# langtech-bsc/quantool

Measured on AMD Instinct MI355X. Metric: quantized weights/sec (GPTQ int4, Llama-3-8B, 512 calib samples), higher is better.
Workload: dtype f32

## Files before the change

include/quantool_amd.h:

```cpp
#ifndef QUANTOOL_AMD_H
#define QUANTOOL_AMD_H

#include <stddef.h>
#include <stdint.h>

#ifdef __cplusplus
extern "C" {
#endif

typedef void* qt_stream_t;

enum qt_status {
    QT_OK = 0,
    QT_ERR_INVALID = -1,
    QT_ERR_NOT_PD = -2,
    QT_ERR_WORKSPACE = -3,
    QT_ERR_HIP = -4,
    QT_ERR_UNSUPPORTED = -5
};

enum qt_dtype { QT_F32 = 0, QT_BF16 = 1, QT_F16 = 2 };

int qt_version(void);
const char* qt_last_error(void);

size_t qt_xtx_workspace_bytes(int64_t n_tokens, int K);
int qt_xtx_accumulate(const void* X, int x_dtype, int64_t n_tokens, int K, int64_t ldx, float* G,
                      void* workspace, size_t workspace_bytes, qt_stream_t stream);

size_t qt_xtx_accumulate_f32_workspace_bytes(int64_t n_tokens, int K);
int qt_xtx_accumulate_f32(const float* X, int64_t n_tokens, int K, int64_t ldx, float* G, void* workspace,
                          size_t workspace_bytes, qt_stream_t stream);

size_t qt_act_stats_workspace_bytes(int64_t n_tokens, int K);
int qt_act_stats_accumulate(const void* X, int x_dtype, int64_t n_tokens, int K, int64_t ldx, float* abs_sum,
                            float* cmin, float* cmax, void* workspace, size_t workspace_bytes,
                            qt_stream_t stream);

size_t qt_hessian_prepare_workspace_bytes(int K);
int qt_hessian_prepare(const float* G, int K, int64_t n_samples, float percdamp,
                       const int32_t* perm, float* A, uint8_t* dead, float* diag_out,
                       void* workspace, size_t workspace_bytes, qt_stream_t stream);
int qt_hessian_prepare_damp(const float* G, int K, int64_t n_samples, float percdamp,
                            const int32_t* perm, float* A, uint8_t* dead, float* diag_out, float* damp_out,
                            void* workspace, size_t workspace_bytes, qt_stream_t stream);
int qt_hessian_diag(const float* G, int K, int64_t n_samples, float* diag_out, qt_stream_t stream);
int qt_argsort_desc(const float* values, int K, int32_t* perm, int32_t* inv, qt_stream_t stream);

size_t qt_cholesky_inverse_upper_workspace_bytes(int K);
int qt_cholesky_inverse_upper(float* A, int K, float* U, int32_t* info, void* workspace,
                              size_t workspace_bytes, qt_stream_t stream);

size_t qt_cholesky_inverse_upper_batched_workspace_bytes(int K, int n_problems);
int qt_cholesky_inverse_upper_batched(float* A, int64_t strideA, int K, float* U, int64_t strideU, int32_t* info,
                                      int n_problems, void* workspace, size_t workspace_bytes, qt_stream_t stream);

int qt_cholesky_inverse_upper_bounded(float* A, int K, float* U, int32_t* info, const float* min_eig_lb,
                                      void* workspace, size_t workspace_bytes, qt_stream_t stream);
int qt_cholesky_inverse_upper_batched_bounded(float* A, int64_t strideA, int K, float* U, int64_t strideU, int32_t* info,
                                              int n_problems, const float* min_eig_lb, void* workspace,
                                              size_t workspace_bytes, qt_stream_t stream);

int qt_group_minmax_qparams(const void* W, int w_dtype, int R, int K, int64_t ldw, int group_size,
                            int symmetric, int num_bits, float* scale, float* zp, float* scale_t,
                            float* zp_t, qt_stream_t stream);

int qt_weight_gather_f32(const void* W, int w_dtype, int R, int K, int64_t ldw, const int32_t* perm,
                         const uint8_t* dead, float* W_f32, qt_stream_t stream);

int qt_weight_gather_qparams(const void* W, int w_dtype, int R, int K, int64_t ldw, const int32_t* perm,
                             const uint8_t* dead, int group_size, int symmetric, int num_bits, float* W_f32, float* scale,
                             float* zp, float* scale_t, float* zp_t, int64_t ld_t, qt_stream_t stream);

size_t qt_gptq_sweep_workspace_bytes(int R, int K, int blocksize);
int qt_gptq_sweep(float* W, int R, int K, const float* U, const float* scale_t, const float* zp_t,
                  int G, const int32_t* g_idx, int blocksize, int num_bits, int8_t* Qt,
                  float* loss, void* workspace, size_t workspace_bytes, qt_stream_t stream);

int qt_gptq_sweep_grouped(float* W, int R, int K, const float* U, int64_t strideU, int n_groups, const int32_t* row_end,
                          const float* scale_t, const float* zp_t, int G, const int32_t* g_idx, int blocksize,
                          int num_bits, int8_t* Qt, float* loss, void* workspace, size_t workspace_bytes,
                          qt_stream_t stream);

int qt_pack_int4(const int8_t* Qt, int R, int K, const int32_t* col_src, int32_t* packed,
                 qt_stream_t stream);

int qt_dequantize(const int8_t* Qt, int R, int K, const int32_t* col_src, const float* scale,
                  const float* zp, int G, const int32_t* g_of_col, void* out, int out_dtype,
                  int64_t ldo, qt_stream_t stream);

size_t qt_awq_weight_mean_workspace_bytes(int R, int K);
int qt_awq_weight_mean_accumulate(const void* W, int w_dtype, int R, int K, int64_t ldw, int group_size,
                                  float* w_sum, void* workspace, size_t workspace_bytes,
                                  qt_stream_t stream);
int qt_awq_scales(const float* x_abs_sum, int64_t n_tokens, const float* w_sum, int64_t n_rows, int K,
                  int n_grid, int duo_scaling, float* scales, qt_stream_t stream);
int qt_symmetrize_lower(float* G, int K, qt_stream_t stream);
size_t qt_awq_loss_workspace_bytes(int R, int K);
int qt_awq_loss(const void* W, int w_dtype, int R, int K, int64_t ldw, const float* s, int group_size,
                int symmetric, int num_bits, const float* Gfull, int64_t n_tokens, int exact, float weight,
                int accumulate, float* loss_out, void* workspace, size_t workspace_bytes, qt_stream_t stream);
size_t qt_awq_losses_workspace_bytes(int R, int K, int n_grid);
int qt_awq_losses(const void* W, int w_dtype, int R, int K, int64_t ldw, const float* scales, int n_grid,
                  int group_size, int symmetric, int num_bits, const float* Gfull, int64_t n_tokens, float weight,
                  int accumulate, float* losses, void* workspace, size_t workspace_bytes, qt_stream_t stream);
int qt_argmin_f32(const float* values, int n, int32_t* index_out, qt_stream_t stream);
int qt_awq_pseudo_quantize(const void* W, int w_dtype, int R, int K, int64_t ldw, const float* s, int group_size,
                           int symmetric, int num_bits, void* out, int64_t ldo, qt_stream_t stream);
int qt_scale_columns(const void* W, int w_dtype, int R, int K, int64_t ldw, const float* s, int divide,
                     void* out, int64_t ldo, qt_stream_t stream);
int qt_rtn_quantize(const void* W, int w_dtype, int R, int K, int64_t ldw, const float* scale,
                    const float* zp, int G, int group_size, int num_bits, int8_t* Qt, qt_stream_t stream);

size_t qt_col_absmax_workspace_bytes(int R, int K);
int qt_col_absmax_accumulate(const void* W, int w_dtype, int R, int K, int64_t ldw, float* wmax,
                             void* workspace, size_t workspace_bytes, qt_stream_t stream);
int qt_smoothquant_scales(const float* cmin, const float* cmax, const float* wmax, int K, float alpha,
                          float* s, qt_stream_t stream);

size_t qt_sgemm_tn_f32_workspace_bytes(int M, int N);
int qt_sgemm_tn_f32(const float* A, int64_t lda, const float* B, int64_t ldb, const float* Cin,
                    int64_t ldcin, float* Cout, int64_t ldcout, int M, int N, int kdim, int skip_zero_k,
                    int mode, int allow_split_k, void* workspace, size_t workspace_bytes, qt_stream_t stream);

int qt_xtx_tile_table_check(int K, int* n_tiles_out, int* chunk_panels_out, int* round_panels_out);

size_t qt_xtx_dot_workspace_bytes(int64_t n_tokens, int K);
int qt_xtx_dot(const void* X, int x_dtype, int64_t n_tokens, int K, int64_t ldx, const float* H, double scale,
               float* out, int accumulate, void* workspace, size_t workspace_bytes, qt_stream_t stream);

size_t qt_gemm3_tn_f32_workspace_bytes(int M, int N, int k);
int qt_gemm3_tn_f32(const float* A, int64_t lda, const float* B, int64_t ldb, float* C, int64_t ldc, int M,
                    int N, int k, int kind, void* workspace, size_t workspace_bytes, qt_stream_t stream);
int qt_gemm3_tn_f32_ex(const float* A, int64_t lda, const float* B, int64_t ldb, float* C, int64_t ldc, int M, int N,
                       int k, int kind, int tri, int tight, int batch, int64_t bsA, int64_t bsB, int64_t bsC,
                       void* workspace, size_t workspace_bytes, qt_stream_t stream);

int qt_gemm3_tn_f16x2(const float* A, int64_t lda, const float* B, int64_t ldb, float* C, int64_t ldc, int M, int N,
                      int k, int kind, int tri, int tight, int batch, int64_t bsA, int64_t bsB, int64_t bsC,
                      const float* bound_a, const float* bound_b, void* workspace, size_t workspace_bytes,
                      qt_stream_t stream);

int qt_gemm3_plan_check(int Tm, int Tn, int c_end, int tri, int* n_items_out, int* n_slabs_out, int* longest_out);
enum qt_act { QT_ACT_SILU = 0 };
#define QT_I8_MID_MAX_M 128
#define QT_I8_MID_K_UNIT 128
#define QT_I8_RING_K_UNIT 128
#define QT_I8_RING_SLOTS 8
#define QT_I8_RING_LEAD 6
#define QT_I8_RING_W4_K_UNIT 128
#define QT_I8_RING_W4_SLOTS 8
#define QT_I8_RING_W4_LEAD 6
#define QT_MOE_I8_WIDE_K_UNIT 128
#define QT_MOE_I8_WIDE_TILE_ROWS 128
#define QT_MOE_I8_WIDE_MAX_E 4096
enum qt_weight_format { QT_W_INT8 = 0, QT_W_INT4_PACKED = 1 };
int qt_quantize_tokens_i8(const void* X, int x_dtype, int64_t M, int K, int64_t ldx, const int32_t* col_perm,
                          int symmetric, int8_t* Xq, float* s_x, int32_t* zp_x, qt_stream_t stream);
int qt_act_mul_quantize_i8(const void* gate, int64_t ldg, const void* up, int64_t ldu, int x_dtype, int64_t M, int K,
                           int act, const int32_t* col_perm, int symmetric, int8_t* Xq, float* s_x, int32_t* zp_x,
                           void* H, int64_t ldh, qt_stream_t stream);
int qt_rmsnorm_quantize_i8(const void* X, int64_t ldx, const void* weight, int x_dtype, int64_t M, int K, float eps,
                           const int32_t* col_perm, int symmetric, int8_t* Xq, float* s_x, int32_t* zp_x,
                           void* Y, int64_t ldy, float* rstd, qt_stream_t stream);
int qt_gemm_i8(const int8_t* Xq, int64_t M, int K, const void* Wq, int w_format, int N, const float* s_x,
               const int32_t* zp_x, const float* s_w, int G, const int32_t* wsum, const void* bias, void* Y,
               int out_dtype, int64_t ldy, qt_stream_t stream);
int qt_gemm_i8_skinny(const int8_t* Xq, int M, int K, const void* Wq, int w_format, int N, const float* s_x,
                      const int32_t* zp_x, const float* s_w, int G, const int32_t* wsum, const void* bias, void* Y,
                      int out_dtype, int64_t ldy, qt_stream_t stream);
int qt_gemm_i8_ring(const int8_t* Xq, int64_t M, int K, const void* Wq, int w_format, int N, const float* s_x,
                    const int32_t* zp_x, const float* s_w, int G, const int32_t* wsum, const void* bias, void* Y,
                    int out_dtype, int64_t ldy, qt_stream_t stream);
int qt_gemm_i8_ring_w4(const int8_t* Xq, int64_t M, int K, const void* Wq, int w_format, int N, const float* s_x,
                       const int32_t* zp_x, const float* s_w, int G, const int32_t* wsum, const void* bias, void* Y,
                       int out_dtype, int64_t ldy, qt_stream_t stream);
int qt_gemm_i8_mid(const int8_t* Xq, int64_t M, int K, const void* Wq, int w_format, int N, const float* s_x,
                   const int32_t* zp_x, const float* s_w, int G, const int32_t* wsum, const void* bias, void* Y,
                   int out_dtype, int64_t ldy, qt_stream_t stream);

int qt_moe_route(const void* top_k_index, int index_is_int64, int64_t T, int k, int E, int32_t* offsets,
                 int32_t* src_token, int32_t* src_slot, int32_t* row_of, qt_stream_t stream);
int qt_gemm_i8_grouped(const int8_t* Xq, int K, const int32_t* row_idx, int64_t R, const int32_t* offsets, int E,
                       const void* Wq, int w_format, int N, const float* s_x, const int32_t* zp_x, const float* s_w,
                       int G, const int32_t* wsum, void* Y, int out_dtype, int64_t ldy, qt_stream_t stream);
int qt_gemm_i8_skinny_grouped(const int8_t* Xq, int K, const int32_t* row_idx, int64_t R, const int32_t* offsets,
                              int E, const void* Wq, int w_format, int N, const float* s_x, const int32_t* zp_x,
                              const float* s_w, int G, const int32_t* wsum, void* Y, int out_dtype, int64_t ldy,
                              qt_stream_t stream);
int qt_gemm_i8_ring_grouped(const int8_t* Xq, int K, const int32_t* row_idx, int64_t R, const int32_t* offsets, int E,
                            const void* Wq, int w_format, int N, const float* s_x, const int32_t* zp_x,
                            const float* s_w, int G, const int32_t* wsum, void* Y, int out_dtype, int64_t ldy,
                            int64_t x_rows, qt_stream_t stream);
int qt_moe_gemm_i8_ring_w4(const int8_t* Xq, int K, const int32_t* row_idx, int64_t R, const int32_t* offsets, int E,
                           const void* Wq, int w_format, int N, const float* s_x, const int32_t* zp_x,
                           const float* s_w, int G, const int32_t* wsum, void* Y, int out_dtype, int64_t ldy,
                           int64_t x_rows, qt_stream_t stream);
int qt_moe_gemm_i8_wide(const int8_t* Xq, int K, const int32_t* row_idx, int64_t R, const int32_t* offsets, int E,
                        const void* Wq, int w_format, int N, const float* s_x, const int32_t* zp_x, const float* s_w,
                        int G, const int32_t* wsum, void* Y, int out_dtype, int64_t ldy, int64_t x_rows,
                        qt_stream_t stream);
int qt_moe_combine(const void* Y, int dtype, int H, int64_t ldy, const int32_t* row_of, const float* weights,
                   int64_t T, int k, void* out, qt_stream_t stream);

int qt_dequantize_weight(const void* Wq, int w_format, int N, int K, const float* s_w, int G, const int8_t* zp_w,
                         const int32_t* g_idx, void* W, int dtype, int64_t ldw, qt_stream_t stream);
int qt_gemm_wq_skinny(const void* X, int x_dtype, int M, int K, int64_t ldx, const void* Wq, int w_format, int N,
                      const float* s_w, int G, const int8_t* zp_w, const int32_t* g_idx, const void* bias, void* Y,
                      int64_t ldy, qt_stream_t stream);

int qt_gemm_wq_stream(const void* X, int x_dtype, int M, int K, int64_t ldx, const void* Wq, int w_format, int N,
                      const float* s_w, int G, const int8_t* zp_w, const int32_t* g_idx, const void* bias, void* Y,
                      int64_t ldy, qt_stream_t stream);
#define QT_WQ_STREAM_MAX_M 128
#define QT_WQ_STREAM_K_UNIT 128
#define QT_WQ_STREAM_MAX_LDX 33554432

int qt_gemm_wq_grouped(const void* X, int x_dtype, int K, int64_t ldx, const int32_t* row_idx, int64_t R,
                       const int32_t* offsets, int E, const void* Wq, int w_format, int N, const float* s_w, int G,
                       const int8_t* zp_w, const int32_t* g_idx, void* Y, int64_t ldy, qt_stream_t stream);

int qt_moe_gemm_wq_wide(const void* X, int x_dtype, int K, int64_t ldx, const int32_t* row_idx, int64_t R,
                        const int32_t* offsets, int E, const void* Wq, int w_format, int N, const float* s_w, int G,
                        const int8_t* zp_w, const int32_t* g_idx, void* Y, int64_t ldy, int64_t x_rows,
                        qt_stream_t stream);
#define QT_MOE_WQ_WIDE_K_UNIT 128
#define QT_MOE_WQ_WIDE_MAX_E 4096
#define QT_MOE_WQ_WIDE_MAX_SLOTS 65535

enum qt_prof_kernel { QT_PROF_XTX = 0, QT_PROF_SWEEP_BLOCK = 1, QT_PROF_NUM_KERNELS = 2 };
int qt_profile_enable(int on);
int qt_profile_read(int kernel_id, double* total_ms, int64_t* launches);

#ifdef __cplusplus
}
#endif
#endif
```

quantool_amd/csrc/cholesky.hip:

```cpp
#include <stdlib.h>
#include <string.h>

#include <map>
#include <tuple>
#include <vector>

#include "common.h"
#include "gemm3_tn.h"
#include "sgemm_tn.h"

namespace {

constexpr int NB = 128;
constexpr int NBO_MAX = 1024;
static int chol_block_env(const char* name) {
    const char* e = getenv(name);
    if (!e) return 0;
    int x = atoi(e) / 128 * 128;
    return x < 128 ? 128 : (x > NBO_MAX ? NBO_MAX : x);
}
struct G3Step {
    int n_items = 0, n_red = 0;
    size_t item_off = 0, red_off = 0;
};
struct CholG3Plan {
    bool any = false;
    std::vector<G3Step> fac, inv;
    char* blob = nullptr;
    size_t blob_bytes = 0;
    int max_slabs = 0;
};

static int chol_g3_min_chunks() {
    const char* on = getenv("QT_CHOL_G3");
    if (on && atoi(on) == 0) return 0;
    const char* e = getenv("QT_CHOL_G3_MIN_CHUNKS");
    const int x = e ? atoi(e) : 64;
    return x < 1 ? 1 : x;
}

static int chol_g3_target_items(int K) {
    const char* e = getenv("QT_G3_TARGET_ITEMS");
    if (e && atoi(e) > 0) return atoi(e);
    return K < 8192 ? 96 : 256;
}

static const CholG3Plan* chol_g3_plan(int K, int NBO, int NBI) {
    static std::mutex m;
    static std::map<std::tuple<int, int, int, int>, CholG3Plan*> plans;
    const int min_chunks = chol_g3_min_chunks();
    const int target_items = chol_g3_target_items(K);
    std::lock_guard<std::mutex> lock(m);
    const auto key = std::make_tuple(K, NBO, NBI, min_chunks * 1024 + target_items);
    auto it = plans.find(key);
    if (it != plans.end()) return it->second;
    CholG3Plan* pl = new CholG3Plan();
    std::vector<char> bytes;
    auto add = [&](int Tm, int Tn, int c_end, int tri) {
        G3Step st;
        if (min_chunks <= 0 || K % 8 != 0 || g3_row_chunks(Tm, Tn, c_end, tri) * G3_CHUNK_ROWS < (long)min_chunks * 128) return st;
        std::vector<G3Item> items;
        std::vector<G3Red> red;
        g3_plan_row(Tm, Tn, c_end, tri, items, red, target_items);
        st.n_items = (int)items.size();
        st.n_red = (int)red.size();
        st.item_off = qt_align_up(bytes.size(), 256);
        bytes.resize(st.item_off + items.size() * sizeof(G3Item));
        memcpy(bytes.data() + st.item_off, items.data(), items.size() * sizeof(G3Item));
        st.red_off = qt_align_up(bytes.size(), 256);
        bytes.resize(st.red_off + red.size() * sizeof(G3Red));
        if (!red.empty()) memcpy(bytes.data() + st.red_off, red.data(), red.size() * sizeof(G3Red));
        for (const G3Red& r : red) pl->max_slabs = pl->max_slabs > r.first + r.count ? pl->max_slabs : r.first + r.count;
        pl->any = true;
        return st;
    };
    for (int J0 = 0; J0 < K; J0 += NBO) {
        const int J1 = (K - J0 < NBO) ? K : J0 + NBO;
        pl->fac.push_back(J0 == 0 ? G3Step() : add((J1 - J0 + 255) / 256, (K - J0 + 255) / 256, J0 / G3_CHUNK_ROWS, 0));
    }
    for (int I0 = 0; I0 < K; I0 += NBI) {
        const int I1 = (K - I0 < NBI) ? K : I0 + NBI;
        pl->inv.push_back(I0 == 0 ? G3Step() : add((I1 - I0 + 255) / 256, (I0 + 255) / 256, I0 / G3_CHUNK_ROWS, 1));
    }
    if (pl->any) {
        pl->blob_bytes = qt_align_up(bytes.size(), 256);
        if (hipHostMalloc((void**)&pl->blob, pl->blob_bytes, hipHostMallocDefault) != hipSuccess) {
            pl->any = false;
            pl->blob = nullptr;
        } else {
            memcpy(pl->blob, bytes.data(), bytes.size());
        }
    }
    if (!pl->any) {
        pl->blob_bytes = 0;
        pl->max_slabs = 0;
        for (G3Step& st : pl->fac) st = G3Step();
        for (G3Step& st : pl->inv) st = G3Step();
    }
    plans[key] = pl;
    return pl;
}
static size_t chol_g3_ws_bytes(const CholG3Plan* pl, int K) {
    if (!pl->any) return 0;
    return 2 * qt_align_up((size_t)3 * K * K * 2, 256) + (size_t)pl->max_slabs * 256 * 256 * 4 + pl->blob_bytes + 256;
}

static const CholG3Plan* chol_blocks(int K, int& NBO, int& NBI) {
    const int eo = chol_block_env("QT_CHOL_NBO"), ei = chol_block_env("QT_CHOL_NBI");
    NBO = eo ? eo : 512;
    NBI = ei ? ei : 512;
    const CholG3Plan* pl = chol_g3_plan(K, NBO, NBI);
    if (pl->any) return pl;
    NBO = eo ? eo : 256;
    NBI = ei ? ei : 256;
    return chol_g3_plan(K, NBO, NBI);
}

constexpr int LDP = NB + 1;

constexpr int LDT = NB + 4;
constexpr int RD_STRIDE = NB * NB + 4 * 32 * 32;

#define QT_SEL4(kb, v0, v1, v2, v3) ((kb) == 0 ? (v0) : (kb) == 1 ? (v1) : (kb) == 2 ? (v2) : (v3))

constexpr int LDA = NB + 4;

__device__ __forceinline__ float readlane_f(float v, int lane) {
    return __int_as_float(__builtin_amdgcn_readlane(__float_as_int(v), lane));
}

__device__ __forceinline__ void mma32_tn(const float* A, int lda, const float* B, int ldb, f32x16& acc,
                                         int l31, int h, bool negate_a) {
#pragma unroll
    for (int kk = 0; kk < 16; ++kk) {
        float a = A[(2 * kk + h) * lda + l31];
        const float b = B[(2 * kk + h) * ldb + l31];
        if (negate_a) a = -a;
        acc = __builtin_amdgcn_mfma_f32_32x32x2f32(a, b, acc, 0, 0, 0);
    }
}

constexpr int POTF2_THREADS = 512, POTF2_WAVES = POTF2_THREADS / 64;
__global__ __launch_bounds__(POTF2_THREADS) void potf2_kernel(const float* P, int64_t ldp, int n,
                                                    float* Rout, int64_t ldr,
                                                    float* __restrict__ Rd, int32_t* info, int col0, int prio,
                                                    int64_t bsP, int64_t bsRd) {
    qt_set_chain_prio(prio);
    if (blockIdx.x) {
        P += (size_t)blockIdx.x * bsP;
        Rout += (size_t)blockIdx.x * bsP;
        Rd += (size_t)blockIdx.x * bsRd;
        info += blockIdx.x;
    }
    extern __shared__ __attribute__((aligned(16))) float sm[];
    float* As = sm;
    float* Xs = sm + NB * LDA;
    const int tid = threadIdx.x, lane = tid & 63;
    const int wave = __builtin_amdgcn_readfirstlane(tid >> 6);
    const int l31 = lane & 31, h = lane >> 5;

    if ((ldp & 3) == 0 && (n & 3) == 0 && (((uintptr_t)P) & 15) == 0) {
        constexpr int NV = NB * NB / 4 / POTF2_THREADS;
        f32x4 v[NV];
#pragma unroll
        for (int r = 0; r < NV; ++r) {
            const int e4 = tid + POTF2_THREADS * r;
            const int i = e4 >> 5, j = (e4 & 31) * 4;
            const int ic = i < n ? i : n - 1, jc = j < n ? j : n - 4;
            v[r] = *(const f32x4*)(P + (size_t)ic * ldp + jc);
        }
#pragma unroll
        for (int r = 0; r < NV; ++r) {
            const int e4 = tid + POTF2_THREADS * r;
            const int i = e4 >> 5, j = (e4 & 31) * 4;
            f32x4 x;
#pragma unroll
            for (int q = 0; q < 4; ++q) x[q] = (i < n && j + q < n) ? v[r][q] : (i == j + q ? 1.0f : 0.0f);
            *(f32x4*)(As + i * LDA + j) = x;
        }
    } else {
        for (int e = tid; e < NB * NB; e += POTF2_THREADS) {
            const int i = e / NB, j = e % NB;
            const int lo = i < j ? i : j, hi = i < j ? j : i;
            float v = (i == j) ? 1.0f : 0.0f;
            if (hi < n) v = P[(size_t)lo * ldp + hi];
            As[i * LDA + j] = v;
        }
    }
    __syncthreads();

    int bad = 0;
#pragma unroll 1
    for (int kb = 0; kb < 4; ++kb) {
        float* Akk = As + (32 * kb) * LDA + 32 * kb;
        if (wave == 0) {
            f32x16 c1, c2;
#pragma unroll
            for (int r = 0; r < 16; ++r) {
                const int i = (r & 3) + 8 * (r >> 2) + 4 * h;
                c1[r] = Akk[i * LDA + l31];
                c2[r] = (i == l31) ? 1.0f : 0.0f;
            }
#pragma unroll
            for (int c = 0; c < 32; ++c) {
                const int rc = (c & 3) + 4 * (c >> 3);
                const int hc = (c >> 2) & 1;
                float piv = readlane_f(c1[rc], c + 32 * hc);
                const bool isbad = !(piv > 0.0f);
                bad = (isbad && bad == 0 && 32 * kb + c < n) ? 32 * kb + c + 1 : bad;
                piv = isbad ? 1.0f : piv;
                float rs = __builtin_amdgcn_rsqf(piv);
                rs = rs * fmaf(-0.5f * piv * rs, rs, 1.5f);
                const bool mine = h == hc;
                const float rr = c1[rc] * rs, zz = c2[rc] * rs;
                c1[rc] = mine ? rr : c1[rc];
                c2[rc] = mine ? zz : c2[rc];
                if (c < 31) {
                    const float a = (mine && l31 > c) ? -rr : 0.0f;
                    const float b1 = (mine && l31 >= c) ? rr : 0.0f, b2 = mine ? zz : 0.0f;
                    c1 = __builtin_amdgcn_mfma_f32_32x32x2f32(a, b1, c1, 0, 0, 0);
                    c2 = __builtin_amdgcn_mfma_f32_32x32x2f32(a, b2, c2, 0, 0, 0);
                }
            }
#pragma unroll
            for (int r = 0; r < 16; ++r) {
                const int i = (r & 3) + 8 * (r >> 2) + 4 * h;
                Akk[i * LDA + l31] = (i <= l31) ? c1[r] : 0.0f;
                Xs[(kb * 32 + l31) * 32 + i] = (i >= l31) ? c2[r] : 0.0f;
            }
        }
        __syncthreads();
        if (kb == 3) break;
        for (int a = kb + 1 + wave; a < 4; a += POTF2_WAVES) {
            f32x16 acc;
#pragma unroll
            for (int r = 0; r < 16; ++r) acc[r] = 0.0f;
            float* Bt = As + (32 * kb) * LDA + 32 * a;
            mma32_tn(Xs + kb * 1024, 32, Bt, LDA, acc, l31, h, false);
#pragma unroll
            for (int r = 0; r < 16; ++r) Bt[((r & 3) + 8 * (r >> 2) + 4 * h) * LDA + l31] = acc[r];
        }
        __syncthreads();
        {
            int t = 0;
            for (int a = kb + 1; a < 4; ++a)
                for (int a2 = a; a2 < 4; ++a2, ++t) {
                    if ((t % POTF2_WAVES) != wave) continue;
                    float* Ct = As + (32 * a) * LDA + 32 * a2;
                    f32x16 acc;
#pragma unroll
                    for (int r = 0; r < 16; ++r) acc[r] = Ct[((r & 3) + 8 * (r >> 2) + 4 * h) * LDA + l31];
                    mma32_tn(As + (32 * kb) * LDA + 32 * a, LDA, As + (32 * kb) * LDA + 32 * a2, LDA, acc, l31, h,
                             true);
#pragma unroll
                    for (int r = 0; r < 16; ++r) Ct[((r & 3) + 8 * (r >> 2) + 4 * h) * LDA + l31] = acc[r];
                }
        }
        __syncthreads();
    }
    if (bad != 0 && tid == 0) atomicCAS(info, 0, col0 + bad);
    const bool vec_out = (ldr & 3) == 0 && (n & 3) == 0 && (((uintptr_t)Rout) & 15) == 0;
    for (int e4 = tid; e4 < NB * NB / 4; e4 += POTF2_THREADS) {
        const int i = e4 >> 5, j = (e4 & 31) * 4;
        f32x4 v = *(const f32x4*)(As + i * LDA + j);
#pragma unroll
        for (int q = 0; q < 4; ++q) v[q] = (j + q >= i) ? v[q] : 0.0f;
        *(f32x4*)(Rd + i * NB + j) = v;
        if (i < n && j + 3 >= i && j < n) {
            if (vec_out) {
                *(f32x4*)(Rout + (size_t)i * ldr + j) = v;
            } else {
#pragma unroll
                for (int q = 0; q < 4; ++q)
                    if (j + q >= i && j + q < n) Rout[(size_t)i * ldr + j + q] = v[q];
            }
        }
    }
    for (int e4 = tid; e4 < 4 * 32 * 32 / 4; e4 += POTF2_THREADS) *(f32x4*)(Rd + NB * NB + 4 * e4) = *(const f32x4*)(Xs + 4 * e4);
}

__global__ __launch_bounds__(256) void trsm_rt_kernel(const float* __restrict__ Rd, int n,
                                                      const float* B, int64_t ldb,
                                                      float* Z, int64_t ldz, int ncols, int prio, int64_t bsRd,
                                                      int64_t bsB) {
    qt_set_chain_prio(prio);
    if (blockIdx.y) {
        Rd += (size_t)blockIdx.y * bsRd;
        B += (size_t)blockIdx.y * bsB;
        Z += (size_t)blockIdx.y * bsB;
    }
    extern __shared__ __attribute__((aligned(16))) float Rs[];
    const int tid = threadIdx.x, lane = tid & 63, wave = tid >> 6;
    const float* D32 = Rs + NB * NB;
    const int l31 = lane & 31, h = lane >> 5;
    const int col = blockIdx.x * 128 + wave * 32 + l31;
    const bool cok = col < ncols;
    const int colc = cok ? col : ncols - 1;

    f32x16 acc[4];
#pragma unroll
    for (int a = 0; a < 4; ++a)
#pragma unroll
        for (int r = 0; r < 16; ++r) {
            const int row = 32 * a + (r & 3) + 8 * (r >> 2) + 4 * h;
            acc[a][r] = (row < n) ? B[(size_t)row * ldb + colc] : 0.0f;
        }
    {
        constexpr int NV = RD_STRIDE / 4 / 256;
        static_assert(NV * 4 * 256 == RD_STRIDE, "whole float4s per thread");
        f32x4 v[NV];
#pragma unroll
        for (int r = 0; r < NV; ++r) v[r] = ((const f32x4*)Rd)[tid + 256 * r];
#pragma unroll
        for (int r = 0; r < NV; ++r) ((f32x4*)Rs)[tid + 256 * r] = v[r];
    }
    __syncthreads();

#pragma unroll
    for (int b = 0; b < 4; ++b) {
        f32x16 zb;
#pragma unroll
        for (int r = 0; r < 16; ++r) zb[r] = 0.0f;
#pragma unroll
        for (int r = 0; r < 16; ++r) {
            const int k = (r & 3) + 8 * (r >> 2) + 4 * h;
            const float av = D32[(b * 32 + k) * 32 + l31];
            zb = __builtin_amdgcn_mfma_f32_32x32x2f32(av, acc[b][r], zb, 0, 0, 0);
        }
        acc[b] = zb;
#pragma unroll
        for (int a = b + 1; a < 4; ++a) {
#pragma unroll
            for (int r = 0; r < 16; ++r) {
                const int k = (r & 3) + 8 * (r >> 2) + 4 * h;
                const float av = -Rs[(32 * b + k) * NB + 32 * a + l31];
                acc[a] = __builtin_amdgcn_mfma_f32_32x32x2f32(av, zb[r], acc[a], 0, 0, 0);
            }
        }
    }
    if (cok) {
#pragma unroll
        for (int a = 0; a < 4; ++a)
#pragma unroll
            for (int r = 0; r < 16; ++r) {
                const int row = 32 * a + (r & 3) + 8 * (r >> 2) + 4 * h;
                if (row < n) Z[(size_t)row * ldz + col] = acc[a][r];
            }
    }
}

__global__ __launch_bounds__(128) void trinv_batched_kernel(const float* __restrict__ Rd_all, int K,
                                                            float* __restrict__ Dinv_all,
                                                            float* __restrict__ Y, int64_t ldy, int64_t bsW, int64_t bsY) {
    if (blockIdx.y) {
        Rd_all += (size_t)blockIdx.y * bsW;
        Dinv_all += (size_t)blockIdx.y * bsW;
        Y += (size_t)blockIdx.y * bsY;
    }
    extern __shared__ __attribute__((aligned(16))) float sm[];
    float* Rt = sm;
    float* Xs = sm + NB * LDT;
    const int b = blockIdx.x;
    const int n = (K - b * NB < NB) ? K - b * NB : NB;
    const float* Rd = Rd_all + (size_t)b * RD_STRIDE;
    const int j = threadIdx.x;
    for (int e = j; e < NB * NB; e += NB) {
        const int i = e / NB, c = e % NB;
        Rt[c * LDT + i] = Rd[e];
    }
    __syncthreads();
    float x0[32], x1[32], x2[32], x3[32];
#pragma unroll
    for (int r = 0; r < 32; ++r) {
        x0[r] = (r == j) ? 1.0f : 0.0f;
        x1[r] = (32 + r == j) ? 1.0f : 0.0f;
        x2[r] = (64 + r == j) ? 1.0f : 0.0f;
        x3[r] = (96 + r == j) ? 1.0f : 0.0f;
    }
#pragma unroll 1
    for (int pb = 3; pb >= 0; --pb) {
#pragma unroll
        for (int pp = 31; pp >= 0; --pp) {
            const int p = 32 * pb + pp;
            const float* rp = Rt + p * LDT;
            const float xp = QT_SEL4(pb, x0[pp], x1[pp], x2[pp], x3[pp]) / rp[p];
            if (pb == 0) x0[pp] = xp;
            if (pb == 1) x1[pp] = xp;
            if (pb == 2) x2[pp] = xp;
            if (pb == 3) x3[pp] = xp;
#define QT_XUPD(arr, a, r_to)                                                 \
    _Pragma("unroll") for (int r4 = 0; r4 < (r_to); r4 += 4) {                 \
        const f32x4 v4 = *(const f32x4*)(rp + 32 * (a) + r4);                 \
        _Pragma("unroll") for (int e = 0; e < 4; ++e)                         \
            if (r4 + e < (r_to)) arr[r4 + e] = fmaf(-v4[e], xp, arr[r4 + e]); \
    }
            if (pb == 0) { QT_XUPD(x0, 0, pp) } else { QT_XUPD(x0, 0, 32) }
            if (pb == 1) { QT_XUPD(x1, 1, pp) } else if (pb > 1) { QT_XUPD(x1, 1, 32) }
            if (pb == 2) { QT_XUPD(x2, 2, pp) } else if (pb > 2) { QT_XUPD(x2, 2, 32) }
            if (pb == 3) { QT_XUPD(x3, 3, pp) }
#undef QT_XUPD
        }
    }
#pragma unroll
    for (int r = 0; r < 32; ++r) {
        Xs[r * LDP + j] = x0[r];
        Xs[(32 + r) * LDP + j] = x1[r];
        Xs[(64 + r) * LDP + j] = x2[r];
        Xs[(96 + r) * LDP + j] = x3[r];
    }
    __syncthreads();
    float* Dinv = Dinv_all + (size_t)b * NB * NB;
    float* Yd = Y + (size_t)(b * NB) * ldy + b * NB;
    for (int e = j; e < NB * NB; e += NB) {
        const int i = e / NB, jj = e % NB;
        const bool in = (i < n && jj < n);
        Dinv[e] = (in && jj >= i) ? Xs[i * LDP + jj] : 0.0f;
        if (in) Yd[(size_t)i * ldy + jj] = (jj <= i) ? Xs[jj * LDP + i] : 0.0f;
    }
}

__global__ __launch_bounds__(256) void trinv_mfma_kernel(const float* __restrict__ Rd_all, int K,
                                                         float* __restrict__ Dinv_all,
                                                         float* __restrict__ Y, int64_t ldy, int64_t bsW, int64_t bsY) {
    if (blockIdx.y) {
        Rd_all += (size_t)blockIdx.y * bsW;
        Dinv_all += (size_t)blockIdx.y * bsW;
        Y += (size_t)blockIdx.y * bsY;
    }
    extern __shared__ __attribute__((aligned(16))) float Rs[];
    const int blk = blockIdx.x;
    const int n = (K - blk * NB < NB) ? K - blk * NB : NB;
    const float* Rd = Rd_all + (size_t)blk * RD_STRIDE;
    const int tid = threadIdx.x, lane = tid & 63, wave = tid >> 6;
    {
        constexpr int NV = RD_STRIDE / 4 / 256;
        f32x4 v[NV];
#pragma unroll
        for (int r = 0; r < NV; ++r) v[r] = ((const f32x4*)Rd)[tid + 256 * r];
#pragma unroll
        for (int r = 0; r < NV; ++r) ((f32x4*)Rs)[tid + 256 * r] = v[r];
    }
    const float* D32 = Rs + NB * NB;
    const int l31 = lane & 31, h = lane >> 5;
    const int col = wave * 32 + l31;

    f32x16 acc[4];
#pragma unroll
    for (int a = 0; a < 4; ++a)
#pragma unroll
        for (int r = 0; r < 16; ++r) {
            const int row = 32 * a + (r & 3) + 8 * (r >> 2) + 4 * h;
            acc[a][r] = (row == col) ? 1.0f : 0.0f;
        }
    __syncthreads();

#pragma unroll
    for (int b = 0; b < 4; ++b) {
        f32x16 zb;
#pragma unroll
        for (int r = 0; r < 16; ++r) zb[r] = 0.0f;
#pragma unroll
        for (int r = 0; r < 16; ++r) {
            const int k = (r & 3) + 8 * (r >> 2) + 4 * h;
            const float av = D32[(b * 32 + k) * 32 + l31];
            zb = __builtin_amdgcn_mfma_f32_32x32x2f32(av, acc[b][r], zb, 0, 0, 0);
        }
        acc[b] = zb;
#pragma unroll
        for (int a = b + 1; a < 4; ++a) {
#pragma unroll
            for (int r = 0; r < 16; ++r) {
                const int k = (r & 3) + 8 * (r >> 2) + 4 * h;
                const float av = -Rs[(32 * b + k) * NB + 32 * a + l31];
                acc[a] = __builtin_amdgcn_mfma_f32_32x32x2f32(av, zb[r], acc[a], 0, 0, 0);
            }
        }
    }
    float* Dinv = Dinv_all + (size_t)blk * NB * NB;
    float* Yd = Y + (size_t)(blk * NB) * ldy + blk * NB;
#pragma unroll
    for (int a = 0; a < 4; ++a)
#pragma unroll
        for (int r = 0; r < 16; ++r) {
            const int row = 32 * a + (r & 3) + 8 * (r >> 2) + 4 * h;
            const bool in = row < n && col < n;
            const float z = (in && row >= col) ? acc[a][r] : 0.0f;
            Dinv[col * NB + row] = z;
            if (in) Yd[(size_t)row * ldy + col] = z;
        }
}

__global__ __launch_bounds__(256) void transpose_lower_block_kernel(const float* __restrict__ Y, int64_t ldy, int w,
                                                                    float* __restrict__ XT, int ldx, int64_t bsY,
                                                                    int64_t bsXT) {
    if (blockIdx.z) {
        Y += (size_t)blockIdx.z * bsY;
        XT += (size_t)blockIdx.z * bsXT;
    }
    __shared__ float tile[32][33];
    const int bx = blockIdx.x * 32, by = blockIdx.y * 32;
    const int tx = threadIdx.x & 31, ty = threadIdx.x >> 5;
    for (int r = ty; r < 32; r += 8) {
        const int m = bx + r, k = by + tx;
        tile[r][tx] = (m < w && k < w && k <= m) ? Y[(size_t)m * ldy + k] : 0.0f;
    }
    __syncthreads();
    for (int r = ty; r < 32; r += 8) {
        const int k = by + r, m = bx + tx;
        if (k < w && m < w) XT[(size_t)k * ldx + m] = tile[tx][r];
    }
}

__global__ __launch_bounds__(256) void flat_reverse_lower_to_upper_kernel(float* __restrict__ U, int K, int64_t bsU) {
    U += (size_t)blockIdx.z * bsU;
    const int j = blockIdx.x * blockDim.x + threadIdx.x;
    const int i = blockIdx.y;
    if (j >= K || j < i) return;
    const size_t e = (size_t)i * K + j;
    const size_t pe = (size_t)(K - 1 - i) * K + (K - 1 - j);
    if (i == j) {
        if (e <= pe) {
            const float t = U[e];
            U[e] = U[pe];
            U[pe] = t;
        }
    } else {
        U[e] = U[pe];
        U[pe] = 0.0f;
    }
}

__global__ __launch_bounds__(256) void identity_if_failed_kernel(float* __restrict__ U, int K,
                                                                 const int32_t* __restrict__ info, int64_t bsU) {
    if (info[blockIdx.z] == 0) return;
    U += (size_t)blockIdx.z * bsU;
    for (int i = blockIdx.x; i < K; i += gridDim.x)
        for (int j = threadIdx.x; j < K; j += blockDim.x) U[(size_t)i * K + j] = (i == j) ? 1.0f : 0.0f;
}

__global__ __launch_bounds__(256) void chol_scales_kernel(const float* __restrict__ A, int64_t bsA, int K,
                                                          const float* __restrict__ min_eig_lb, int32_t* __restrict__ e,
                                                          int32_t* __restrict__ info) {
    __shared__ float red[256];
    const int b = blockIdx.x, nprob = gridDim.x;
    const float* Ab = A + (size_t)b * bsA;
    float m = 0.0f;
    for (int i = threadIdx.x; i < K; i += 256) m = fmaxf(m, Ab[(size_t)i * K + i]);
    red[threadIdx.x] = m;
    __syncthreads();
    for (int s = 128; s > 0; s >>= 1) {
        if ((int)threadIdx.x < s) red[threadIdx.x] = fmaxf(red[threadIdx.x], red[threadIdx.x + s]);
        __syncthreads();
    }
    if (threadIdx.x == 0) {
        auto clampe = [](float t) { return (int)fminf(fmaxf(t, (float)-G3_E_MAX), (float)G3_E_MAX); };
        const float d = red[0], lb = min_eig_lb[b];
        e[b] = (d > 0.0f && d < 3.0e38f) ? clampe(3.0f - ceilf(0.5f * log2f(d))) : 0;
        if (lb > 0.0f && lb < 3.0e38f) {
            e[nprob + b] = clampe(3.0f - ceilf(-0.5f * log2f(lb)));
        } else {
            e[nprob + b] = 0;
            info[b] = K + 1;
        }
    }
}

}

static size_t chol_problem_ws_bytes(int K, const CholG3Plan* g3) {
    const size_t nb = (K + NB - 1) / NB;
    const size_t split = (size_t)2048 * NB * NB * 4 + (size_t)NBO_MAX * K * 4;
    size_t n = (size_t)NB * K * 4 + (size_t)NBO_MAX * K * 4 + (size_t)NBO_MAX * NBO_MAX * 4 + nb * (NB * NB + RD_STRIDE) * 4 + split + 256;
    if (g3->any) n += 2 * qt_align_up((size_t)3 * K * K * 2, 256) + (size_t)g3->max_slabs * 256 * 256 * 4 + 256;
    return qt_align_up(n, 256);
}

extern "C" size_t qt_cholesky_inverse_upper_batched_workspace_bytes(int K, int n_problems) {
    if (K <= 0 || n_problems <= 0) return 0;
    int nbo_, nbi_;
    const CholG3Plan* g3 = chol_blocks(K, nbo_, nbi_);
    return (size_t)n_problems * chol_problem_ws_bytes(K, g3) + g3->blob_bytes + 512;
}

extern "C" size_t qt_cholesky_inverse_upper_workspace_bytes(int K) {
    return qt_cholesky_inverse_upper_batched_workspace_bytes(K, 1);
}

static int chol_run(float* A, int64_t strideA, int K, float* U, int64_t strideU, int32_t* info, int nprob, void* workspace,
                    size_t workspace_bytes, hipStream_t stream, const float* min_eig_lb = nullptr) {
    bool f16x2 = min_eig_lb != nullptr;
    if (const char* e = getenv("QT_CHOL_PLANES")) {
        if (strcmp(e, "bf16x3") == 0) f16x2 = false;
        else if (strcmp(e, "f16x2") == 0) {
            QT_CHECK_ARG(min_eig_lb, "qt_cholesky_inverse_upper: QT_CHOL_PLANES=f16x2 needs a bound on lambda_min (the _bounded entry points)");
        } else {
            QT_CHECK_ARG(false, "qt_cholesky_inverse_upper: QT_CHOL_PLANES=%s (bf16x3 | f16x2)", e);
        }
    }
    const size_t need = qt_cholesky_inverse_upper_batched_workspace_bytes(K, nprob);
    if (!workspace || workspace_bytes < need) {
        qt_set_error("qt_cholesky_inverse_upper: workspace %zu < required %zu", workspace_bytes, need);
        return QT_ERR_WORKSPACE;
    }
    const int nblk = (K + NB - 1) / NB;
    char* ws = (char*)qt_align_up((size_t)workspace, 256);
    int NBO, NBI;
    const CholG3Plan* g3 = chol_blocks(K, NBO, NBI);
    const size_t prob_bytes = chol_problem_ws_bytes(K, g3);
    const int64_t sW = (int64_t)(prob_bytes / 4);
    const int64_t sA = nprob > 1 ? strideA : 0, sU = nprob > 1 ? strideU : 0;
    float* T = (float*)ws;
    float* TI = T + (size_t)NB * K;
    float* XT = TI + (size_t)NBO_MAX * K;
    float* Rd = XT + (size_t)NBO_MAX * NBO_MAX;
    float* Dinv = Rd + (size_t)nblk * RD_STRIDE;
    float* split_ws = Dinv + (size_t)nblk * NB * NB;
    const size_t split_ws_bytes = (size_t)2048 * NB * NB * 4 + (size_t)NBO_MAX * K * 4;
    unsigned short *Rpl = nullptr, *Ypl = nullptr;
    float* g3_slabs = nullptr;
    char* g3_tab = nullptr;
    const int64_t plane_stride = (int64_t)K * K;
    if (g3->any) {
        char* q = (char*)qt_align_up((size_t)((char*)split_ws + split_ws_bytes), 256);
        Rpl = (unsigned short*)q;
        q += qt_align_up((size_t)3 * K * K * 2, 256);
        Ypl = (unsigned short*)q;
        q += qt_align_up((size_t)3 * K * K * 2, 256);
        g3_slabs = (float*)q;
        g3_tab = (char*)qt_align_up((size_t)(ws + (size_t)nprob * prob_bytes), 256);
        QT_HIP(hipMemcpyAsync(g3_tab, g3->blob, g3->blob_bytes, hipMemcpyHostToDevice, stream));
    }
    f16x2 = f16x2 && g3->any;
    int32_t* eR = f16x2 ? (int32_t*)(Rpl + 2 * plane_stride) : nullptr;
    int32_t* eY = f16x2 ? eR + nprob : nullptr;
    static_assert(2 * SG_MAX_BATCH * sizeof(int32_t) <= (size_t)NB * NB * 2, "the exponents fit the smallest third plane");
    auto g3_row = [&](const G3Step& st, const unsigned short* Bplanes, int col_a0, int col_b0, int M, int N, float* C,
                      int64_t bsC, int mode) -> int {
        G3Args a;
        a.Apl = Rpl;
        a.Bpl = Bplanes;
        a.plane_stride = plane_stride;
        a.ld = K;
        a.rowA0 = a.rowB0 = 0;
        a.colA0 = col_a0;
        a.colB0 = col_b0;
        a.colmax = K;
        a.M = M;
        a.N = N;
        a.C = C;
        a.ldc = K;
        a.mode = mode;
        a.slabs = g3_slabs;
        a.items = (const G3Item*)(g3_tab + st.item_off);
        a.n_items = st.n_items;
        a.red = (const G3Red*)(g3_tab + st.red_off);
        a.n_red = st.n_red;
        a.batch = nprob;
        a.bsApl = a.bsBpl = sW * 2;
        a.bsC = bsC;
        a.bsSlabs = sW;
        if (f16x2) {
            a.planes = G3_F16X2;
            a.eA = eR;
            a.eB = Bplanes == Rpl ? eR : eY;
        }
        return qt_gemm3_launch(a, stream);
    };
    auto sgemm = [&](SgemmArgs& g, int64_t bsA_, int64_t bsB_, int64_t bsC_) -> int {
        g.batch = nprob;
        g.bsA = bsA_;
        g.bsB = bsB_;
        g.bsCin = g.bsCout = bsC_;
        g.bs_split = sW;
        return qt_sgemm_tn(g, stream);
    };
    float* Y = U;
    const int64_t sY = sU;
    const size_t inv_lds = (size_t)(NB * LDT + NB * LDP) * sizeof(float);
    const size_t potf2_lds = (size_t)(NB * LDA + 4 * 32 * 32) * sizeof(float);
    static QtOncePerDevice lds_attr;
    QT_HIP(lds_attr.run([&] {
        hipError_t e = hipFuncSetAttribute((const void*)potf2_kernel, hipFuncAttributeMaxDynamicSharedMemorySize,
                                           (int)potf2_lds);
        if (e == hipSuccess)
            e = hipFuncSetAttribute((const void*)trsm_rt_kernel, hipFuncAttributeMaxDynamicSharedMemorySize,
                                    (int)(RD_STRIDE * sizeof(float)));
        if (e == hipSuccess)
            e = hipFuncSetAttribute((const void*)trinv_batched_kernel, hipFuncAttributeMaxDynamicSharedMemorySize,
                                    (int)inv_lds);
        if (e == hipSuccess)
            e = hipFuncSetAttribute((const void*)trinv_mfma_kernel, hipFuncAttributeMaxDynamicSharedMemorySize,
                                    (int)(RD_STRIDE * sizeof(float)));
        return e;
    }));
    QT_HIP(hipMemsetAsync(info, 0, sizeof(int32_t) * nprob, stream));
    const int prio = qt_chain_prio();
    if (f16x2) {
        hipLaunchKernelGGL(chol_scales_kernel, dim3(nprob), dim3(256), 0, stream, (const float*)A, sA, K, min_eig_lb, eR, info);
        QT_LAUNCH_CHECK();
    }

    for (int J0 = 0, Jb = 0; J0 < K; J0 += NBO, ++Jb) {
        const int J1 = (K - J0 < NBO) ? K : J0 + NBO;
        if (g3->any && J0 > 0) {
            const G3Step& st = g3->fac[Jb];
            float* C = A + (size_t)J0 * K + J0;
            if (st.n_items > 0) {
                int rc = g3_row(st, Rpl, J0, J0, J1 - J0, K - J0, C, sA, G3_SUB);
                if (rc) return rc;
            } else {
                SgemmArgs g;
                g.A = A + J0; g.lda = K;
                g.B = A + J0; g.ldb = K;
                g.Cin = C; g.ldcin = K;
                g.Cout = C; g.ldcout = K;
                g.M = J1 - J0; g.N = K - J0; g.kdim = J0; g.k_mode = SG_K_FULL; g.mode = SG_MODE_SUB;
                g.split_ws = split_ws; g.split_ws_bytes = split_ws_bytes;
                int rc = sgemm(g, sA, sA, sA);
                if (rc) return rc;
            }
        }
        for (int j0 = J0; j0 < J1; j0 += NB) {
            const int j = j0 / NB, nbj = (K - j0 < NB) ? K - j0 : NB;
            float* Ajj = A + (size_t)j0 * K + j0;
            if (j0 > J0) {
                SgemmArgs g;
                g.A = A + (size_t)J0 * K + j0; g.lda = K;
                g.B = A + (size_t)J0 * K + j0; g.ldb = K;
                g.Cin = Ajj; g.ldcin = K;
                g.Cout = Ajj; g.ldcout = K;
                g.M = nbj; g.N = K - j0; g.kdim = j0 - J0; g.k_mode = SG_K_FULL; g.mode = SG_MODE_SUB;
                int rc = sgemm(g, sA, sA, sA);
                if (rc) return rc;
            }
            hipLaunchKernelGGL(potf2_kernel, dim3(nprob), dim3(POTF2_THREADS), potf2_lds, stream, (const float*)Ajj, (int64_t)K, nbj,
                               Ajj, (int64_t)K, Rd + (size_t)j * RD_STRIDE, info, j0, prio, sA, sW);
            QT_LAUNCH_CHECK();
            const int rest = K - j0 - nbj;
            if (rest > 0) {
                hipLaunchKernelGGL(trsm_rt_kernel, dim3((rest + 127) / 128, nprob), dim3(256), RD_STRIDE * sizeof(float),
                                   stream, (const float*)(Rd + (size_t)j * RD_STRIDE), nbj, (const float*)(Ajj + nbj),
                                   (int64_t)K, Ajj + nbj, (int64_t)K, rest, prio, sW, sA);
                QT_LAUNCH_CHECK();
            }
        }
        const int rem = K - J1;
        if (g3->any) {
            if (rem > 0) {
                int rc = f16x2 ? qt_split2h_launch(A + (size_t)J0 * K + J0, K, J1 - J0, K - J0, Rpl + (size_t)J0 * K + J0, K,
                                                   plane_stride, 0, 0, 0, eR, stream, nprob, sA, sW * 2)
                               : qt_split3_launch(A + (size_t)J0 * K + J0, K, J1 - J0, K - J0, Rpl + (size_t)J0 * K + J0, K,
                                                  plane_stride, 0, 0, 0, stream, nprob, sA, sW * 2);
                if (rc) return rc;
            }
        } else if (rem > 0) {
            SgemmArgs g;
            g.A = A + (size_t)J0 * K + J1; g.lda = K;
            g.B = A + (size_t)J0 * K + J1; g.ldb = K;
            g.Cin = A + (size_t)J1 * K + J1; g.ldcin = K;
            g.Cout = A + (size_t)J1 * K + J1; g.ldcout = K;
            g.M = rem; g.N = rem; g.kdim = J1 - J0; g.k_mode = SG_K_FULL; g.mode = SG_MODE_SUB;
            g.upper_only = 1;
            int rc = sgemm(g, sA, sA, sA);
            if (rc) return rc;
        }
    }
    {
        const char* e = getenv("QT_CHOL_TRINV");
        if (e && strcmp(e, "div") == 0)
            hipLaunchKernelGGL(trinv_batched_kernel, dim3(nblk, nprob), dim3(NB), inv_lds, stream, (const float*)Rd, K, Dinv, Y,
                               (int64_t)K, sW, sY);
        else
            hipLaunchKernelGGL(trinv_mfma_kernel, dim3(nblk, nprob), dim3(256), RD_STRIDE * sizeof(float), stream,
                               (const float*)Rd, K, Dinv, Y, (int64_t)K, sW, sY);
    }
    QT_LAUNCH_CHECK();
    for (int I0 = 0, Ib = 0; I0 < K; I0 += NBI, ++Ib) {
        const int I1 = (K - I0 < NBI) ? K : I0 + NBI;
        const int Wi = I1 - I0;
        for (int i0 = I0 + NB; i0 < I1; i0 += NB) {
            const int i = i0 / NB, nbi = (K - i0 < NB) ? K - i0 : NB;
            SgemmArgs g;
            g.A = A + (size_t)I0 * K + i0; g.lda = K;
            g.B = Y + (size_t)I0 * K + I0; g.ldb = K;
            g.Cin = nullptr; g.ldcin = 0;
            g.Cout = T; g.ldcout = K;
            g.M = nbi; g.N = i0 - I0; g.kdim = i0 - I0; g.k_mode = SG_K_FROM_N0; g.mode = SG_MODE_SET;
            int rc = sgemm(g, sA, sY, sW);
            if (rc) return rc;
            SgemmArgs t;
            t.A = Dinv + (size_t)i * NB * NB; t.lda = NB;
            t.B = T; t.ldb = K;
            t.Cin = nullptr; t.ldcin = 0;
            t.Cout = Y + (size_t)i0 * K + I0; t.ldcout = K;
            t.M = nbi; t.N = i0 - I0; t.kdim = nbi; t.k_mode = SG_K_FULL; t.mode = SG_MODE_NEG;
            rc = sgemm(t, sW, sW, sY);
            if (rc) return rc;
        }
        auto split_row = [&]() -> int {
            if (!g3->any || I1 >= K) return QT_OK;
            if (f16x2)
                return qt_split2h_launch(Y + (size_t)I0 * K, K, Wi, I1, Ypl + (size_t)I0 * K, K, plane_stride, 1, I0, 0, eY,
                                         stream, nprob, sY, sW * 2);
            return qt_split3_launch(Y + (size_t)I0 * K, K, Wi, I1, Ypl + (size_t)I0 * K, K, plane_stride, 1, I0, 0, stream,
                                    nprob, sY, sW * 2);
        };
        if (I0 == 0) {
            int rc0 = split_row();
            if (rc0) return rc0;
            continue;
        }
        int rc;
        if (g3->any && g3->inv[Ib].n_items > 0) {
            rc = g3_row(g3->inv[Ib], Ypl, I0, 0, Wi, I0, TI, sW, G3_SET);
        } else {
            SgemmArgs g;
            g.A = A + I0; g.lda = K;
            g.B = Y; g.ldb = K;
            g.Cin = nullptr; g.ldcin = 0;
            g.Cout = TI; g.ldcout = K;
            g.M = Wi; g.N = I0; g.kdim = I0; g.k_mode = SG_K_FROM_N0; g.mode = SG_MODE_SET;
            g.split_ws = split_ws; g.split_ws_bytes = split_ws_bytes;
            rc = sgemm(g, sA, sY, sW);
        }
        if (rc) return rc;
        hipLaunchKernelGGL(transpose_lower_block_kernel, dim3((Wi + 31) / 32, (Wi + 31) / 32, nprob), dim3(256), 0, stream,
                           (const float*)(Y + (size_t)I0 * K + I0), (int64_t)K, Wi, XT, NBO_MAX, sY, sW);
        QT_LAUNCH_CHECK();
        SgemmArgs t;
        t.A = XT; t.lda = NBO_MAX;
        t.B = TI; t.ldb = K;
        t.Cin = nullptr; t.ldcin = 0;
        t.Cout = Y + (size_t)I0 * K; t.ldcout = K;
        t.M = Wi; t.N = I0; t.kdim = Wi; t.k_mode = SG_K_FULL; t.mode = SG_MODE_NEG;
        rc = sgemm(t, sW, sW, sY);
        if (rc) return rc;
        rc = split_row();
        if (rc) return rc;
    }
    hipLaunchKernelGGL(flat_reverse_lower_to_upper_kernel, dim3((K + 255) / 256, K, nprob), dim3(256), 0, stream, U, K, sU);
    QT_LAUNCH_CHECK();
    hipLaunchKernelGGL(identity_if_failed_kernel, dim3(K < 1024 ? K : 1024, 1, nprob), dim3(256), 0, stream, U, K,
                       (const int32_t*)info, sU);
    QT_LAUNCH_CHECK();
    return QT_OK;
}

extern "C" int qt_cholesky_inverse_upper(float* A, int K, float* U, int32_t* info, void* workspace,
                                         size_t workspace_bytes, qt_stream_t stream_) {
    QT_CHECK_ARG(K > 0 && A && U && info, "qt_cholesky_inverse_upper: bad arguments");
    return chol_run(A, 0, K, U, 0, info, 1, workspace, workspace_bytes, (hipStream_t)stream_);
}

extern "C" int qt_cholesky_inverse_upper_batched(float* A, int64_t strideA, int K, float* U, int64_t strideU, int32_t* info,
                                                 int n_problems, void* workspace, size_t workspace_bytes,
                                                 qt_stream_t stream_) {
    QT_CHECK_ARG(K > 0 && A && U && info && n_problems >= 1 && n_problems <= SG_MAX_BATCH,
                 "qt_cholesky_inverse_upper_batched: bad arguments (1 <= n_problems <= %d)", SG_MAX_BATCH);
    QT_CHECK_ARG(n_problems == 1 || (strideA >= (int64_t)K * K && strideU >= (int64_t)K * K && strideA % 4 == 0 && strideU % 4 == 0),
                 "qt_cholesky_inverse_upper_batched: strides must be multiples of 4 elements and >= K*K");
    return chol_run(A, strideA, K, U, strideU, info, n_problems, workspace, workspace_bytes, (hipStream_t)stream_);
}

extern "C" int qt_cholesky_inverse_upper_bounded(float* A, int K, float* U, int32_t* info, const float* min_eig_lb,
                                                 void* workspace, size_t workspace_bytes, qt_stream_t stream_) {
    QT_CHECK_ARG(K > 0 && A && U && info && min_eig_lb, "qt_cholesky_inverse_upper_bounded: bad arguments");
    return chol_run(A, 0, K, U, 0, info, 1, workspace, workspace_bytes, (hipStream_t)stream_, min_eig_lb);
}

extern "C" int qt_cholesky_inverse_upper_batched_bounded(float* A, int64_t strideA, int K, float* U, int64_t strideU,
                                                         int32_t* info, int n_problems, const float* min_eig_lb,
                                                         void* workspace, size_t workspace_bytes, qt_stream_t stream_) {
    QT_CHECK_ARG(K > 0 && A && U && info && min_eig_lb && n_problems >= 1 && n_problems <= SG_MAX_BATCH,
                 "qt_cholesky_inverse_upper_batched_bounded: bad arguments (1 <= n_problems <= %d)", SG_MAX_BATCH);
    QT_CHECK_ARG(n_problems == 1 || (strideA >= (int64_t)K * K && strideU >= (int64_t)K * K && strideA % 4 == 0 && strideU % 4 == 0),
                 "qt_cholesky_inverse_upper_batched_bounded: strides must be multiples of 4 elements and >= K*K");
    return chol_run(A, strideA, K, U, strideU, info, n_problems, workspace, workspace_bytes, (hipStream_t)stream_, min_eig_lb);
}
```

quantool_amd/csrc/gemm3_tn.h:

```cpp
#pragma once
#include <vector>

#include "common.h"

constexpr int G3_CHUNK_ROWS = 64;

struct G3Item {
    int tile;
    int c_lo;
    int c_hi;
    int slab;
};
struct G3Red {
    int tile;
    int first;
    int count;
    int pad;
};

enum { G3_SUB = 0, G3_SET = 1, G3_ADD = 2 };

enum { G3_BF16X3 = 0, G3_F16X2 = 1 };
constexpr int G3_E_MAX = 40;

struct G3Args {
    const unsigned short* Apl;
    const unsigned short* Bpl;
    int64_t plane_stride;
    int64_t ld;
    int64_t rowA0, rowB0;
    int colA0, colB0;
    int colmax;
    int M, N;
    float* C;
    int64_t ldc;
    int64_t ldB = 0, plane_strideB = 0;
    int colmaxB = 0;
    int mode;
    float* slabs;
    const G3Item* items;
    int n_items;
    const G3Red* red;
    int n_red;
    int batch = 1;
    int64_t bsApl = 0, bsBpl = 0, bsC = 0, bsSlabs = 0;
    int planes = G3_BF16X3;
    const int32_t* eA = nullptr;
    const int32_t* eB = nullptr;
};

int qt_gemm3_launch(const G3Args& a, hipStream_t stream);

int qt_split3_launch(const float* src, int64_t ld_src, int rows, int cols, unsigned short* planes, int64_t ld_pl,
                     int64_t plane_stride, int mask_upper, int row_g0, int col_g0, hipStream_t stream, int batch = 1,
                     int64_t bs_src = 0, int64_t bs_planes = 0);

int qt_split2h_launch(const float* src, int64_t ld_src, int rows, int cols, unsigned short* planes, int64_t ld_pl,
                      int64_t plane_stride, int mask_upper, int row_g0, int col_g0, const int32_t* e, hipStream_t stream,
                      int batch = 1, int64_t bs_src = 0, int64_t bs_planes = 0);

int g3_scale_exponent(float bound);

long g3_row_chunks(int Tm, int Tn, int c_end, int tri);
void g3_plan_row(int Tm, int Tn, int c_end, int tri, std::vector<G3Item>& items, std::vector<G3Red>& red, int target_items = 0);
```

quantool_amd/csrc/gemm3_tn.hip:

```cpp
#include <math.h>
#include <stdlib.h>
#include <string.h>

#include <algorithm>
#include <map>
#include <mutex>
#include <type_traits>

#include "gemm3_tn.h"
#include "ring_pipe.h"

namespace {

constexpr int RING = 8;
constexpr int CH_ROWS = G3_CHUNK_ROWS;
constexpr int CH_UNITS = 6 * (CH_ROWS / UT);
constexpr int TRING = 3;
constexpr int TRI_BYTES = 3 * UNIT_BYTES;
constexpr int TRI_DMA = 6;
constexpr int DRING = 4;
constexpr int DUO_BYTES = 2 * UNIT_BYTES;
constexpr int DUO_DMA = 4;
constexpr int DUO_LEAD = 2;
enum { LOOP_CHUNK = 0, LOOP_TRI = 1, LOOP_DUO = 2 };
static_assert(CH_ROWS / UT == 4, "the phase code below recomputes the source pointers every 4 units");
constexpr unsigned PA_BITS = 2u | (0u << 2) | (1u << 4) | (1u << 6) | (0u << 8) | (0u << 10);
constexpr unsigned PB_BITS = 0u | (2u << 2) | (1u << 4) | (0u << 6) | (1u << 8) | (0u << 10);
constexpr int g3_plane_a(int pr) { return (PA_BITS >> (2 * pr)) & 3u; }
constexpr int g3_plane_b(int pr) { return (PB_BITS >> (2 * pr)) & 3u; }

struct G3Params {
    const char* Apl;
    const char* Bpl;
    int64_t plane_bytes, plane_bytesB;
    int64_t ld2, ld2B;
    int64_t rowA0, rowB0;
    int colA0, colB0, colmax, colmaxB;
    int M, N;
    float* C;
    int64_t ldc;
    float* slabs;
    const G3Item* items;
    int64_t bsA_bytes, bsB_bytes, bsC, bsSlabs;
    const int32_t* eA;
    const int32_t* eB;
};

template <int MODE, int LOOP>
__global__ __launch_bounds__(NTHREADS, 2) void gemm3_kernel(G3Params p) {
    constexpr bool TRI = LOOP == LOOP_TRI;
    __shared__ __attribute__((aligned(16))) char ring[LOOP == LOOP_DUO ? DRING * DUO_BYTES : TRI ? TRING * TRI_BYTES : RING * UNIT_BYTES];
    const int tid = threadIdx.x;
    const int lane = tid & 63;
    const int wave = __builtin_amdgcn_readfirstlane(tid >> 6);
    const int wave_m = wave >> 2, wave_n = wave & 3;
    const bool group_b = wave >= 4;

    if (blockIdx.y) {
        p.Apl += (size_t)blockIdx.y * p.bsA_bytes;
        p.Bpl += (size_t)blockIdx.y * p.bsB_bytes;
        p.C += (size_t)blockIdx.y * p.bsC;
        p.slabs += (size_t)blockIdx.y * p.bsSlabs;
    }
    const G3Item* itp = p.items + blockIdx.x;
    const int it_tile = __builtin_amdgcn_readfirstlane(itp->tile);
    const int c_lo = __builtin_amdgcn_readfirstlane(itp->c_lo);
    const int c_hi = __builtin_amdgcn_readfirstlane(itp->c_hi);
    const int slab_idx = __builtin_amdgcn_readfirstlane(itp->slab);
    const int ti = it_tile >> 16, tj = it_tile & 0xFFFF;
    const int nu = (c_hi - c_lo) * (LOOP != LOOP_CHUNK ? CH_ROWS / UT : CH_UNITS);

    const int rsub = lane >> 4;
    const int lch = (lane & 15) ^ (rsub << 2);
    const int trow = 4 * (wave & 3) + rsub;
    int colA = p.colA0 + ti * BT + (wave >> 2) * 128 + lch * 8;
    int colB = p.colB0 + tj * BT + (wave >> 2) * 128 + lch * 8;
    colA = colA > p.colmax - 8 ? p.colmax - 8 : colA;
    colB = colB > p.colmaxB - 8 ? p.colmaxB - 8 : colB;
    const unsigned voffA = (unsigned)((size_t)trow * (size_t)p.ld2 + (size_t)colA * 2);
    const unsigned voffB = (unsigned)((size_t)trow * (size_t)p.ld2B + (size_t)colB * 2);
    const unsigned ring_lds = (unsigned)(size_t)(QT_LDS char*)ring;
    const unsigned dst_wave =
        __builtin_amdgcn_readfirstlane(ring_lds + (wave >> 2) * 4096 + (wave & 3) * 1024);

    const int64_t ustride = (int64_t)UT * p.ld2, ustrideB = (int64_t)UT * p.ld2B;

    const int g = lane >> 4, il = lane & 15, q = il >> 2, pp = il & 3;
    const int rowpart = (8 * (g >> 1) + q) * 256 + 32 * (g & 1) + 8 * pp;
    int aoff[4], boff[2];
#pragma unroll
    for (int mi = 0; mi < 4; ++mi) aoff[mi] = wave_m * 4096 + rowpart + 64 * (mi ^ q);
#pragma unroll
    for (int ni = 0; ni < 2; ++ni)
        boff[ni] = (2 + (wave_n >> 1)) * 4096 + rowpart + 64 * ((((wave_n & 1) << 1) + ni) ^ q);

    f32x16 acc[4][2];
#pragma unroll
    for (int mi = 0; mi < 4; ++mi)
#pragma unroll
        for (int ni = 0; ni < 2; ++ni)
#pragma unroll
            for (int r = 0; r < 16; ++r) acc[mi][ni][r] = 0.0f;

    if constexpr (LOOP == LOOP_DUO) {
        const char* runA = p.Apl + (p.rowA0 + (int64_t)c_lo * CH_ROWS) * p.ld2;
        const char* runB = p.Bpl + (p.rowB0 + (int64_t)c_lo * CH_ROWS) * p.ld2B;
        auto issue2 = [&](int slot) {
            const unsigned d = dst_wave + (unsigned)slot * DUO_BYTES;
#pragma unroll
            for (int pl = 0; pl < 2; ++pl)
                glds16_pair2(voffA, voffB, runA + pl * p.plane_bytes, runB + pl * p.plane_bytesB, d + pl * UNIT_BYTES,
                             d + pl * UNIT_BYTES + 8192);
            runA += ustride;
            runB += ustrideB;
        };
        s16x8 fa[2][4], fb[2][2];
        auto phase = [&](auto slot_c, int u) {
            constexpr int S = decltype(slot_c)::value;
            constexpr int ISLOT = (S + DUO_LEAD) % DRING;
            const char* base = ring + S * DUO_BYTES;
#pragma unroll
            for (int pl = 0; pl < 2; ++pl) {
#pragma unroll
                for (int mi = 0; mi < 4; ++mi) fa[pl][mi] = tr_load8(base + pl * UNIT_BYTES + aoff[mi]);
#pragma unroll
                for (int ni = 0; ni < 2; ++ni) fb[pl][ni] = tr_load8(base + pl * UNIT_BYTES + boff[ni]);
            }
            if (u + DUO_LEAD < nu) issue2(ISLOT);
            ring_drain_wait<DUO_DMA, DUO_LEAD>(nu - u - 2);
            ring_sync_math([&] {
                s16x8 fbs[2];
#pragma unroll
                for (int ni = 0; ni < 2; ++ni)
                    fbs[ni] = __builtin_bit_cast(s16x8, __builtin_bit_cast(f16x8, fb[0][ni]) * (_Float16)2048.0f);
                ring_mma32<true>(fa[1], fb[0], acc);
                ring_mma32<true>(fa[0], fb[1], acc);
                ring_mma32<true>(fa[0], fbs, acc);
            });
        };
        if (nu > 0) {
            issue2(0);
            issue2(1);
            wait_vmcnt<DUO_DMA*(DUO_LEAD - 1)>();
            ring_stagger_begin(group_b);
            for (int u = 0; u < nu; u += DRING) ring_body<DRING>(phase, u);
            ring_stagger_end(group_b);
        }
        const int es = -(11 + p.eA[blockIdx.y] + p.eB[blockIdx.y]);
        const float unscale = __builtin_bit_cast(float, (unsigned)(127 + (es < -126 ? -126 : es > 127 ? 127 : es)) << 23);
#pragma unroll
        for (int mi = 0; mi < 4; ++mi)
#pragma unroll
            for (int ni = 0; ni < 2; ++ni)
#pragma unroll
                for (int r = 0; r < 16; ++r) acc[mi][ni][r] *= unscale;
    } else if constexpr (TRI) {
        const char* runA = p.Apl + (p.rowA0 + (int64_t)c_lo * CH_ROWS) * p.ld2;
        const char* runB = p.Bpl + (p.rowB0 + (int64_t)c_lo * CH_ROWS) * p.ld2B;
        auto issue3 = [&](int slot) {
            const unsigned d = dst_wave + (unsigned)slot * TRI_BYTES;
#pragma unroll
            for (int pl = 0; pl < 3; ++pl)
                glds16_pair2(voffA, voffB, runA + pl * p.plane_bytes, runB + pl * p.plane_bytesB, d + pl * UNIT_BYTES,
                             d + pl * UNIT_BYTES + 8192);
            runA += ustride;
            runB += ustrideB;
        };
        s16x8 fa[3][4], fb[3][2];
        auto phase = [&](auto slot_c, int u) {
            constexpr int S = decltype(slot_c)::value;
            constexpr int ISLOT = (S + 2) % TRING;
            const bool more = u + 2 < nu;
            if (group_b && more) issue3(ISLOT);
            const char* base = ring + S * TRI_BYTES;
#pragma unroll
            for (int pl = 0; pl < 3; ++pl) {
#pragma unroll
                for (int mi = 0; mi < 4; ++mi) fa[pl][mi] = tr_load8(base + pl * UNIT_BYTES + aoff[mi]);
#pragma unroll
                for (int ni = 0; ni < 2; ++ni) fb[pl][ni] = tr_load8(base + pl * UNIT_BYTES + boff[ni]);
            }
            if (group_b) ring_drain_wait<TRI_DMA, 2>(nu - u - 2);
            ring_sync_math(
                [&] {
                    if (!group_b && more) issue3(ISLOT);
                },
                [&] {
                    ring_mma32<false>(fa[g3_plane_a(0)], fb[g3_plane_b(0)], acc);
                    ring_mma32<false>(fa[g3_plane_a(1)], fb[g3_plane_b(1)], acc);
                    ring_mma32<false>(fa[g3_plane_a(2)], fb[g3_plane_b(2)], acc);
                    ring_mma32<false>(fa[g3_plane_a(3)], fb[g3_plane_b(3)], acc);
                    ring_mma32<false>(fa[g3_plane_a(4)], fb[g3_plane_b(4)], acc);
                    ring_mma32<false>(fa[g3_plane_a(5)], fb[g3_plane_b(5)], acc);
                },
                [&] {
                    if (!group_b) ring_drain_wait<TRI_DMA, 2>(nu - u - 2);
                });
        };
        if (nu > 0) {
            issue3(0);
            issue3(1);
            wait_vmcnt<TRI_DMA>();
            ring_stagger_begin(group_b);
            int u = 0;
            for (; u + TRING <= nu; u += TRING) ring_body<TRING>(phase, u);
            if (u < nu) phase(std::integral_constant<int, 0>{}, u);
            if (u + 1 < nu) phase(std::integral_constant<int, 1>{}, u + 1);
            ring_stagger_end(group_b);
        }
    } else {
        constexpr int LEAD = 6;
        auto unit_src = [&](int i, const char*& a, const char*& b) {
            const int g = i >> 2, j = i & 3;
            const int c = g / 6, pr = g - 6 * c;
            const int64_t plA = (PA_BITS >> (2 * pr)) & 3u, plB = (PB_BITS >> (2 * pr)) & 3u;
            const int64_t row = (int64_t)(c_lo + c) * CH_ROWS + j * UT;
            a = p.Apl + plA * p.plane_bytes + (p.rowA0 + row) * p.ld2;
            b = p.Bpl + plB * p.plane_bytesB + (p.rowB0 + row) * p.ld2B;
        };
        auto issue = [&](int i, int slot) {
            const char *a, *b;
            unit_src(i, a, b);
            const unsigned d = dst_wave + (unsigned)slot * UNIT_BYTES;
            glds16_pair2(voffA, voffB, a, b, d, d + 8192);
        };
        const char *runA = nullptr, *runB = nullptr;

        s16x8 fa[4], fb[2];
        auto drain_wait = [&](int u) {
            ring_drain_wait<2, LEAD>(nu - u - 2);
        };
        auto phase = [&](auto slot_c, auto steady_c, int u) {
            constexpr int S = decltype(slot_c)::value;
            constexpr bool STEADY = decltype(steady_c)::value;
            constexpr int ISLOT = (S + LEAD) & (RING - 1);
            const char* base = ring + S * UNIT_BYTES;
#pragma unroll
            for (int mi = 0; mi < 4; ++mi) fa[mi] = tr_load8(base + aoff[mi]);
#pragma unroll
            for (int ni = 0; ni < 2; ++ni) fb[ni] = tr_load8(base + boff[ni]);
            if (STEADY) {
                if (S == 2 || S == 6) unit_src(u + LEAD, runA, runB);
                const unsigned d = dst_wave + (unsigned)ISLOT * UNIT_BYTES;
                glds16_pair2(voffA, voffB, runA, runB, d, d + 8192);
                runA += ustride;
                runB += ustrideB;
                wait_vmcnt<2 * (LEAD - 1)>();
            } else if (u + LEAD < nu) {
                issue(u + LEAD, ISLOT);
                wait_vmcnt<2 * (LEAD - 1)>();
            } else {
                drain_wait(u);
            }
            ring_sync_math([&] { ring_mma32<false>(fa, fb, acc); });
        };
        auto body8 = [&](auto steady_c, int u) {
            ring_body<8>([&](auto slot_c, int uu) { phase(slot_c, steady_c, uu); }, u);
        };

        if (nu > 0) {
#pragma unroll
            for (int i = 0; i < LEAD; ++i) issue(i, i);
            wait_vmcnt<2 * (LEAD - 1)>();
            ring_stagger_begin(group_b);
            unit_src(LEAD, runA, runB);
            int u = 0;
            for (; u + 8 + LEAD <= nu; u += 8) body8(std::true_type{}, u);
            for (; u + 8 <= nu; u += 8) body8(std::false_type{}, u);
            ring_stagger_end(group_b);
        }
    }

    const int jl = lane & 31, ih = 4 * (lane >> 5);
    if (slab_idx < 0) {
#pragma unroll
        for (int mi = 0; mi < 4; ++mi)
#pragma unroll
            for (int ni = 0; ni < 2; ++ni) {
                const int gj = tj * BT + wave_n * 64 + ni * 32 + jl;
#pragma unroll
                for (int r = 0; r < 16; ++r) {
                    const int gi = ti * BT + wave_m * 128 + mi * 32 + (r & 3) + 8 * (r >> 2) + ih;
                    if (gi < p.M && gj < p.N) {
                        float* dst = p.C + (size_t)gi * p.ldc + gj;
                        if (MODE == G3_SUB) *dst = *dst - acc[mi][ni][r];
                        else if (MODE == G3_ADD) *dst = *dst + acc[mi][ni][r];
                        else *dst = acc[mi][ni][r];
                    }
                }
            }
    } else {
        float* slab = p.slabs + (size_t)slab_idx * (size_t)(BT * BT);
#pragma unroll
        for (int mi = 0; mi < 4; ++mi)
#pragma unroll
            for (int ni = 0; ni < 2; ++ni)
#pragma unroll
                for (int r = 0; r < 16; ++r) {
                    const int i_loc = wave_m * 128 + mi * 32 + (r & 3) + 8 * (r >> 2) + ih;
                    const int j_loc = wave_n * 64 + ni * 32 + jl;
                    slab[i_loc * BT + j_loc] = acc[mi][ni][r];
                }
    }
}

__global__ __launch_bounds__(256) void gemm3_reduce_kernel(const float* __restrict__ slabs,
                                                           const G3Red* __restrict__ red, float* C, int64_t ldc,
                                                           int M, int N, int mode, int64_t bsSlabs, int64_t bsC) {
    if (blockIdx.z) {
        slabs += (size_t)blockIdx.z * bsSlabs;
        C += (size_t)blockIdx.z * bsC;
    }
    const G3Red t = red[blockIdx.x];
    const int ti = t.tile >> 16, tj = t.tile & 0xFFFF;
    const int part = blockIdx.y;
    const size_t tile_elems = (size_t)BT * BT;
    for (int e = threadIdx.x; e < 16 * (BT / 4); e += blockDim.x) {
        const int i_loc = part * 16 + e / (BT / 4);
        const int j_loc = (e % (BT / 4)) * 4;
        const int gi = ti * BT + i_loc, gj = tj * BT + j_loc;
        if (gi >= M || gj >= N) continue;
        f32x4 s = {0.f, 0.f, 0.f, 0.f};
        for (int sp = 0; sp < t.count; ++sp) {
            const f32x4 v = *(const f32x4*)(slabs + (size_t)(t.first + sp) * tile_elems + (size_t)i_loc * BT + j_loc);
            s += v;
        }
        float* dst = C + (size_t)gi * ldc + gj;
        if (gj + 3 < N && (ldc & 3) == 0 && (((uintptr_t)C) & 15) == 0) {
            if (mode == G3_SUB) {
                f32x4 o = *(f32x4*)dst;
                o -= s;
                *(f32x4*)dst = o;
            } else if (mode == G3_ADD) {
                f32x4 o = *(f32x4*)dst;
                o += s;
                *(f32x4*)dst = o;
            } else {
                *(f32x4*)dst = s;
            }
        } else {
            for (int c = 0; c < 4 && gj + c < N; ++c)
                dst[c] = (mode == G3_SUB) ? dst[c] - s[c] : (mode == G3_ADD) ? dst[c] + s[c] : s[c];
        }
    }
}

__device__ __forceinline__ unsigned short bf16_bits_rne(float v) {
    return __builtin_bit_cast(unsigned short, (__bf16)v);
}

__global__ __launch_bounds__(256) void split3_kernel(const float* __restrict__ src, int64_t ld_src, int cols,
                                                     unsigned short* __restrict__ planes, int64_t ld_pl,
                                                     int64_t plane_stride, int mask_upper, int row_g0, int col_g0,
                                                     int64_t bs_src, int64_t bs_planes) {
    if (blockIdx.z) {
        src += (size_t)blockIdx.z * bs_src;
        planes += (size_t)blockIdx.z * bs_planes;
    }
    const int c4 = (blockIdx.x * 256 + threadIdx.x) * 4;
    const int r = blockIdx.y;
    if (c4 >= cols) return;
    f32x4 v = *(const f32x4*)(src + (size_t)r * ld_src + c4);
    typedef __attribute__((ext_vector_type(4))) unsigned short u16x4;
    u16x4 hi, mid, lo;
#pragma unroll
    for (int e = 0; e < 4; ++e) {
        float x = v[e];
        if (mask_upper && col_g0 + c4 + e > row_g0 + r) x = 0.0f;
        const unsigned short h = bf16_bits_rne(x);
        const float r1 = x - qt_bf16_to_f32(h);
        const unsigned short m = bf16_bits_rne(r1);
        const float r2 = r1 - qt_bf16_to_f32(m);
        hi[e] = h;
        mid[e] = m;
        lo[e] = bf16_bits_rne(r2);
    }
    unsigned short* dst = planes + (size_t)r * ld_pl + c4;
    *(u16x4*)dst = hi;
    *(u16x4*)(dst + plane_stride) = mid;
    *(u16x4*)(dst + 2 * plane_stride) = lo;
}

__global__ __launch_bounds__(256) void split2h_kernel(const float* __restrict__ src, int64_t ld_src, int cols,
                                                      unsigned short* __restrict__ planes, int64_t ld_pl,
                                                      int64_t plane_stride, int mask_upper, int row_g0, int col_g0,
                                                      int64_t bs_src, int64_t bs_planes, const int32_t* __restrict__ e) {
    const int ex = e[blockIdx.z];
    if (blockIdx.z) {
        src += (size_t)blockIdx.z * bs_src;
        planes += (size_t)blockIdx.z * bs_planes;
    }
    const int c4 = (blockIdx.x * 256 + threadIdx.x) * 4;
    const int r = blockIdx.y;
    if (c4 >= cols) return;
    const float scale = __builtin_bit_cast(float, (unsigned)(127 + (ex < -G3_E_MAX ? -G3_E_MAX : ex > G3_E_MAX ? G3_E_MAX : ex)) << 23);
    f32x4 v = *(const f32x4*)(src + (size_t)r * ld_src + c4);
    typedef __attribute__((ext_vector_type(4))) unsigned short u16x4;
    u16x4 hi, lo;
#pragma unroll
    for (int q = 0; q < 4; ++q) {
        float x = v[q] * scale;
        if (mask_upper && col_g0 + c4 + q > row_g0 + r) x = 0.0f;
        const _Float16 h = (_Float16)x;
        const float r1 = x - (float)h;
        hi[q] = __builtin_bit_cast(unsigned short, h);
        lo[q] = __builtin_bit_cast(unsigned short, (_Float16)(r1 * 2048.0f));
    }
    unsigned short* dst = planes + (size_t)r * ld_pl + c4;
    *(u16x4*)dst = hi;
    *(u16x4*)(dst + plane_stride) = lo;
}

}

int qt_gemm3_launch(const G3Args& a, hipStream_t stream) {
    if (a.n_items <= 0) return QT_OK;
    QT_CHECK_ARG(a.ld % 8 == 0 && a.colmax >= 8, "qt_gemm3_launch: plane pitch %lld must be a multiple of 8", (long long)a.ld);
    QT_CHECK_ARG(((uintptr_t)a.Apl & 15) == 0 && ((uintptr_t)a.Bpl & 15) == 0 && (a.plane_stride % 8) == 0,
                 "qt_gemm3_launch: planes must be 16-byte aligned");
    QT_CHECK_ARG((uint64_t)a.ld * 2 * UT + (uint64_t)a.colmax * 2 < ((uint64_t)1 << 32), "qt_gemm3_launch: pitch too large");
    G3Params p;
    p.Apl = (const char*)a.Apl;
    p.Bpl = (const char*)a.Bpl;
    p.plane_bytes = a.plane_stride * 2;
    p.ld2 = a.ld * 2;
    p.plane_bytesB = (a.plane_strideB ? a.plane_strideB : a.plane_stride) * 2;
    p.ld2B = (a.ldB ? a.ldB : a.ld) * 2;
    p.colmaxB = a.colmaxB ? a.colmaxB : a.colmax;
    QT_CHECK_ARG(p.ld2B % 16 == 0 && p.colmaxB >= 8 && (p.plane_bytesB % 16) == 0 &&
                     (uint64_t)p.ld2B * UT + (uint64_t)p.colmaxB * 2 < ((uint64_t)1 << 32),
                 "qt_gemm3_launch: B-side pitch %lld / columns %d unsupported", (long long)(p.ld2B / 2), p.colmaxB);
    p.rowA0 = a.rowA0;
    p.rowB0 = a.rowB0;
    p.colA0 = a.colA0;
    p.colB0 = a.colB0;
    p.colmax = a.colmax;
    p.M = a.M;
    p.N = a.N;
    p.C = a.C;
    p.ldc = a.ldc;
    p.slabs = a.slabs;
    p.items = a.items;
    const int nb = a.batch > 1 ? a.batch : 1;
    QT_CHECK_ARG(nb <= 65535 && (a.bsApl % 8) == 0 && (a.bsBpl % 8) == 0, "qt_gemm3_launch: batch %d / plane strides unsupported", nb);
    p.bsA_bytes = a.bsApl * 2;
    p.bsB_bytes = a.bsBpl * 2;
    p.bsC = a.bsC;
    p.bsSlabs = a.bsSlabs;
    QT_CHECK_ARG(a.planes == G3_BF16X3 || (a.planes == G3_F16X2 && a.eA && a.eB),
                 "qt_gemm3_launch: plane mode %d needs its scale exponents", a.planes);
    p.eA = a.eA;
    p.eB = a.eB;
    const dim3 grid(a.n_items, nb);
    const char* loop_env = getenv("QT_G3_LOOP");
    const bool chunk_loop = loop_env && strcmp(loop_env, "chunk") == 0;
    auto launch = [&](auto loop_c) {
        constexpr int LOOP = decltype(loop_c)::value;
        if (a.mode == G3_SUB) hipLaunchKernelGGL((gemm3_kernel<G3_SUB, LOOP>), grid, dim3(NTHREADS), 0, stream, p);
        else if (a.mode == G3_ADD) hipLaunchKernelGGL((gemm3_kernel<G3_ADD, LOOP>), grid, dim3(NTHREADS), 0, stream, p);
        else hipLaunchKernelGGL((gemm3_kernel<G3_SET, LOOP>), grid, dim3(NTHREADS), 0, stream, p);
    };
    if (a.planes == G3_F16X2) launch(std::integral_constant<int, LOOP_DUO>{});
    else if (chunk_loop) launch(std::integral_constant<int, LOOP_CHUNK>{});
    else launch(std::integral_constant<int, LOOP_TRI>{});
    QT_LAUNCH_CHECK();
    if (a.n_red > 0) {
        hipLaunchKernelGGL(gemm3_reduce_kernel, dim3(a.n_red, 16, nb), dim3(256), 0, stream, (const float*)a.slabs, a.red,
                           a.C, a.ldc, a.M, a.N, a.mode, a.bsSlabs, a.bsC);
        QT_LAUNCH_CHECK();
    }
    return QT_OK;
}

int qt_split3_launch(const float* src, int64_t ld_src, int rows, int cols, unsigned short* planes, int64_t ld_pl,
                     int64_t plane_stride, int mask_upper, int row_g0, int col_g0, hipStream_t stream, int batch,
                     int64_t bs_src, int64_t bs_planes) {
    if (rows <= 0 || cols <= 0) return QT_OK;
    QT_CHECK_ARG(cols % 4 == 0 && ld_src % 4 == 0 && ld_pl % 4 == 0 && plane_stride % 4 == 0 &&
                     ((uintptr_t)src & 15) == 0 && ((uintptr_t)planes & 7) == 0,
                 "qt_split3_launch: columns / pitches must be multiples of 4 and the pointers aligned");
    QT_CHECK_ARG(bs_src % 4 == 0 && bs_planes % 4 == 0, "qt_split3_launch: batch strides must be multiples of 4");
    hipLaunchKernelGGL(split3_kernel, dim3((cols / 4 + 255) / 256, rows, batch > 1 ? batch : 1), dim3(256), 0, stream, src,
                       ld_src, cols, planes, ld_pl, plane_stride, mask_upper, row_g0, col_g0, bs_src, bs_planes);
    QT_LAUNCH_CHECK();
    return QT_OK;
}

int qt_split2h_launch(const float* src, int64_t ld_src, int rows, int cols, unsigned short* planes, int64_t ld_pl,
                      int64_t plane_stride, int mask_upper, int row_g0, int col_g0, const int32_t* e, hipStream_t stream,
                      int batch, int64_t bs_src, int64_t bs_planes) {
    if (rows <= 0 || cols <= 0) return QT_OK;
    QT_CHECK_ARG(e && cols % 4 == 0 && ld_src % 4 == 0 && ld_pl % 4 == 0 && plane_stride % 4 == 0 &&
                     ((uintptr_t)src & 15) == 0 && ((uintptr_t)planes & 7) == 0,
                 "qt_split2h_launch: columns / pitches must be multiples of 4 and the pointers aligned");
    QT_CHECK_ARG(bs_src % 4 == 0 && bs_planes % 4 == 0, "qt_split2h_launch: batch strides must be multiples of 4");
    hipLaunchKernelGGL(split2h_kernel, dim3((cols / 4 + 255) / 256, rows, batch > 1 ? batch : 1), dim3(256), 0, stream, src,
                       ld_src, cols, planes, ld_pl, plane_stride, mask_upper, row_g0, col_g0, bs_src, bs_planes, e);
    QT_LAUNCH_CHECK();
    return QT_OK;
}

long g3_row_chunks(int Tm, int Tn, int c_end, int tri) {
    constexpr int TRI_STEP = 256 / G3_CHUNK_ROWS;
    long total = 0;
    for (int tj = 0; tj < Tn; ++tj) total += (long)Tm * std::max(0, c_end - (tri ? TRI_STEP * tj : 0));
    return total;
}

void g3_plan_row(int Tm, int Tn, int c_end, int tri, std::vector<G3Item>& items, std::vector<G3Red>& red, int target_items) {
    constexpr int TRI_STEP = 256 / G3_CHUNK_ROWS;
    items.clear();
    red.clear();
    const long total = g3_row_chunks(Tm, Tn, c_end, tri);
    const int cap = target_items > 0 && target_items < NUM_CU ? target_items : NUM_CU;
    auto count_items = [&](int per) {
        long n_items = 0;
        for (int tj = 0; tj < Tn; ++tj) {
            const int n = c_end - (tri ? TRI_STEP * tj : 0);
            if (n > 0) n_items += (long)Tm * ((n + per - 1) / per);
        }
        return n_items;
    };
    int per = std::max(2, (int)((total + cap - 1) / cap));
    while (count_items(per) > cap && per < c_end) ++per;
    int next_slab = 0;
    for (int ti = 0; ti < Tm; ++ti)
        for (int tj = 0; tj < Tn; ++tj) {
            const int lo = tri ? TRI_STEP * tj : 0, n = c_end - lo;
            if (n <= 0) continue;
            const int pieces = (n + per - 1) / per;
            const int tile = (ti << 16) | tj;
            if (pieces == 1) {
                items.push_back({tile, lo, c_end, -1});
                continue;
            }
            red.push_back({tile, next_slab, pieces, 0});
            for (int s = 0; s < pieces; ++s) {
                const int a = lo + (int)((long)n * s / pieces), b = lo + (int)((long)n * (s + 1) / pieces);
                items.push_back({tile, a, b, next_slab++});
            }
        }
    std::stable_sort(items.begin(), items.end(),
                     [](const G3Item& x, const G3Item& y) { return (x.c_hi - x.c_lo) > (y.c_hi - y.c_lo); });
    static const bool deal = [] { const char* e = getenv("QT_G3_DEAL"); return !(e && atoi(e) == 0); }();
    if (deal && items.size() > 8) {
        std::vector<int> starts;
        for (const G3Item& it : items) starts.push_back(it.c_lo);
        std::sort(starts.begin(), starts.end());
        starts.erase(std::unique(starts.begin(), starts.end()), starts.end());
        const int P = (int)starts.size();
        const int g = P >= 8 ? 1 : 8 / P;
        std::vector<std::vector<G3Item>> cls(8);
        for (const G3Item& it : items) {
            const int rank = (int)(std::lower_bound(starts.begin(), starts.end(), it.c_lo) - starts.begin());
            const int tj = it.tile & 0xFFFF;
            cls[(rank * g + (g > 1 ? tj % g : 0)) % 8].push_back(it);
        }
        std::vector<G3Item> dealt;
        dealt.reserve(items.size());
        for (size_t q = 0; dealt.size() < items.size(); ++q)
            for (int x = 0; x < 8; ++x)
                if (q < cls[x].size()) dealt.push_back(cls[x][q]);
        items.swap(dealt);
    }
}

int g3_scale_exponent(float bound) {
    if (!(bound > 0.0f) || bound > 3.0e38f) return 0;
    int x;
    const float m = frexpf(bound, &x);
    const int ceil_log2 = m == 0.5f ? x - 1 : x;
    const int e = 3 - ceil_log2;
    return e < -G3_E_MAX ? -G3_E_MAX : e > G3_E_MAX ? G3_E_MAX : e;
}

constexpr size_t G3_TEST_TABLE_BYTES = (size_t)1 << 20;
constexpr size_t G3_TEST_SLACK = 1024;
static size_t g3_test_layout(int M, int N, int k, int64_t& ldp, size_t& planes_bytes, size_t& slabs_bytes) {
    ldp = (int64_t)qt_align_up((size_t)std::max(M, N), 256);
    planes_bytes = (size_t)3 * k * ldp * 2;
    slabs_bytes = (size_t)2 * NUM_CU * BT * BT * 4;
    return 2 * planes_bytes + slabs_bytes + G3_TEST_TABLE_BYTES + G3_TEST_SLACK;
}

extern "C" size_t qt_gemm3_tn_f32_workspace_bytes(int M, int N, int k) {
    if (M <= 0 || N <= 0 || k <= 0) return 0;
    int64_t ldp;
    size_t pb, sb;
    return g3_test_layout(M, N, k, ldp, pb, sb);
}

static int g3_test_run(const char* who, const float* A, int64_t lda, const float* B, int64_t ldb, float* C, int64_t ldc,
                       int M, int N, int k, int kind, int tri, int tight, int batch, int64_t bsA, int64_t bsB, int64_t bsC,
                       void* workspace, size_t workspace_bytes, hipStream_t stream, const float* bound_a = nullptr,
                       const float* bound_b = nullptr) {
    const bool f16x2 = bound_a && bound_b;
    constexpr size_t EXP_BYTES = 256;
    QT_CHECK_ARG(!f16x2 || batch <= 32, "%s: at most 32 problems with bounds", who);
    QT_CHECK_ARG(A && B && C && M > 0 && N > 0 && k > 0 && k % 128 == 0, "%s: k=%d must be a positive multiple of 128", who, k);
    QT_CHECK_ARG(M % 4 == 0 && N % 4 == 0 && lda % 4 == 0 && ldb % 4 == 0, "%s: M, N, lda, ldb must be multiples of 4", who);
    QT_CHECK_ARG(batch >= 1 && bsA % 4 == 0 && bsB % 4 == 0, "%s: batch %d / strides unsupported", who, batch);
    int64_t ldp;
    size_t pb, sb;
    const size_t need = g3_test_layout(M, N, k, ldp, pb, sb);
    if (!workspace || workspace_bytes < need * (size_t)batch) {
        qt_set_error("%s: workspace %zu < required %zu", who, workspace_bytes, need * (size_t)batch);
        return QT_ERR_WORKSPACE;
    }
    const size_t per = need - G3_TEST_SLACK;
    if (tight) ldp = (int64_t)qt_align_up((size_t)std::max(M, N), 8);
    const int64_t plane_stride = (int64_t)k * ldp;
    char* ws = (char*)qt_align_up((size_t)workspace, 256);
    unsigned short* Apl = (unsigned short*)ws;
    unsigned short* Bpl = (unsigned short*)(ws + pb);
    float* slabs = (float*)(ws + 2 * pb);
    char* tab = ws + 2 * pb + sb;
    int32_t* exps = (int32_t*)(tab + G3_TEST_TABLE_BYTES - EXP_BYTES);
    if (f16x2) {
        int32_t host_e[64] = {0};
        for (int b = 0; b < batch; ++b) {
            QT_CHECK_ARG(bound_a[b] > 0.0f && bound_b[b] > 0.0f, "%s: bounds must be positive", who);
            host_e[b] = g3_scale_exponent(bound_a[b]);
            host_e[32 + b] = g3_scale_exponent(bound_b[b]);
        }
        QT_HIP(hipStreamSynchronize(stream));
        QT_HIP(hipMemcpy(exps, host_e, sizeof(host_e), hipMemcpyHostToDevice));
    }
    for (int b = 0; b < batch; ++b) QT_HIP(hipMemsetAsync(ws + (size_t)b * per, 0, 2 * pb, stream));
    int rc = f16x2 ? qt_split2h_launch(A, lda, k, M, Apl, ldp, plane_stride, 0, 0, 0, exps, stream, batch, bsA, (int64_t)(per / 2))
                   : qt_split3_launch(A, lda, k, M, Apl, ldp, plane_stride, 0, 0, 0, stream, batch, bsA, (int64_t)(per / 2));
    if (rc) return rc;
    rc = f16x2 ? qt_split2h_launch(B, ldb, k, N, Bpl, ldp, plane_stride, 0, 0, 0, exps + 32, stream, batch, bsB, (int64_t)(per / 2))
               : qt_split3_launch(B, ldb, k, N, Bpl, ldp, plane_stride, 0, 0, 0, stream, batch, bsB, (int64_t)(per / 2));
    if (rc) return rc;
    const int Tm = (M + BT - 1) / BT, Tn = (N + BT - 1) / BT, nch = k / CH_ROWS;
    constexpr int TRI_STEP = 256 / G3_CHUNK_ROWS;
    QT_CHECK_ARG(!tri || TRI_STEP * (Tn - 1) < nch, "%s: tri needs k > 256 * (tile columns - 1)", who);
    std::vector<G3Item> items;
    std::vector<G3Red> red;
    if (kind == 0) {
        for (int ti = 0; ti < Tm; ++ti)
            for (int tj = 0; tj < Tn; ++tj) items.push_back({(ti << 16) | tj, tri ? TRI_STEP * tj : 0, nch, -1});
    } else {
        int next = 0;
        for (int ti = 0; ti < Tm; ++ti)
            for (int tj = 0; tj < Tn; ++tj) {
                const int lo = tri ? TRI_STEP * tj : 0, n = nch - lo;
                const int pieces = std::min(n / 2, std::max(1, 2 * NUM_CU / (Tm * Tn)));
                red.push_back({(ti << 16) | tj, next, pieces, 0});
                for (int s = 0; s < pieces; ++s)
                    items.push_back({(ti << 16) | tj, lo + (int)((long)n * s / pieces), lo + (int)((long)n * (s + 1) / pieces), next++});
            }
        QT_CHECK_ARG((size_t)next * BT * BT * 4 <= sb, "%s: too many tiles for the test face", who);
    }
    const size_t ib = items.size() * sizeof(G3Item), rb = red.size() * sizeof(G3Red);
    QT_CHECK_ARG(qt_align_up(ib, 256) + rb <= G3_TEST_TABLE_BYTES - EXP_BYTES, "%s: table too large for the test face", who);
    QT_HIP(hipStreamSynchronize(stream));
    QT_HIP(hipMemcpy(tab, items.data(), ib, hipMemcpyHostToDevice));
    if (rb) QT_HIP(hipMemcpy(tab + qt_align_up(ib, 256), red.data(), rb, hipMemcpyHostToDevice));
    G3Args g;
    g.Apl = Apl;
    g.Bpl = Bpl;
    g.plane_stride = plane_stride;
    g.ld = ldp;
    g.rowA0 = g.rowB0 = 0;
    g.colA0 = g.colB0 = 0;
    g.colmax = (int)ldp;
    g.M = M;
    g.N = N;
    g.C = C;
    g.ldc = ldc;
    g.mode = kind == 0 ? G3_SUB : G3_SET;
    g.slabs = slabs;
    g.items = (const G3Item*)tab;
    g.n_items = (int)items.size();
    g.red = (const G3Red*)(tab + qt_align_up(ib, 256));
    g.n_red = (int)red.size();
    g.batch = batch;
    g.bsApl = g.bsBpl = (int64_t)(per / 2);
    g.bsC = bsC;
    g.bsSlabs = (int64_t)(per / 4);
    if (f16x2) {
        g.planes = G3_F16X2;
        g.eA = exps;
        g.eB = exps + 32;
    }
    return qt_gemm3_launch(g, stream);
}

extern "C" int qt_gemm3_tn_f32(const float* A, int64_t lda, const float* B, int64_t ldb, float* C, int64_t ldc, int M,
                               int N, int k, int kind, void* workspace, size_t workspace_bytes, qt_stream_t stream_) {
    return g3_test_run("qt_gemm3_tn_f32", A, lda, B, ldb, C, ldc, M, N, k, kind, 0, 0, 1, 0, 0, 0, workspace, workspace_bytes,
                       (hipStream_t)stream_);
}

extern "C" int qt_gemm3_tn_f32_ex(const float* A, int64_t lda, const float* B, int64_t ldb, float* C, int64_t ldc, int M,
                                  int N, int k, int kind, int tri, int tight, int batch, int64_t bsA, int64_t bsB,
                                  int64_t bsC, void* workspace, size_t workspace_bytes, qt_stream_t stream_) {
    return g3_test_run("qt_gemm3_tn_f32_ex", A, lda, B, ldb, C, ldc, M, N, k, kind, tri, tight, batch, bsA, bsB, bsC, workspace,
                       workspace_bytes, (hipStream_t)stream_);
}

extern "C" int qt_gemm3_tn_f16x2(const float* A, int64_t lda, const float* B, int64_t ldb, float* C, int64_t ldc, int M,
                                 int N, int k, int kind, int tri, int tight, int batch, int64_t bsA, int64_t bsB,
                                 int64_t bsC, const float* bound_a, const float* bound_b, void* workspace,
                                 size_t workspace_bytes, qt_stream_t stream_) {
    QT_CHECK_ARG(bound_a && bound_b, "qt_gemm3_tn_f16x2: bounds are required");
    return g3_test_run("qt_gemm3_tn_f16x2", A, lda, B, ldb, C, ldc, M, N, k, kind, tri, tight, batch, bsA, bsB, bsC, workspace,
                       workspace_bytes, (hipStream_t)stream_, bound_a, bound_b);
}

constexpr int XF_CHUNK = 8192;

static int64_t xf_pitch(int K) { return (int64_t)qt_align_up((size_t)K, 256); }

extern "C" size_t qt_xtx_accumulate_f32_workspace_bytes(int64_t n_tokens, int K) {
    if (n_tokens <= 0 || K <= 0) return 0;
    const int nt = (K + BT - 1) / BT;
    return (size_t)3 * XF_CHUNK * xf_pitch(K) * 2 + qt_align_up((size_t)nt * (nt + 1) / 2 * sizeof(G3Item), 256) * 2 + 1024;
}

extern "C" int qt_xtx_accumulate_f32(const float* X, int64_t n_tokens, int K, int64_t ldx, float* G, void* workspace,
                                     size_t workspace_bytes, qt_stream_t stream_) {
    hipStream_t stream = (hipStream_t)stream_;
    QT_CHECK_ARG(X && G && K > 0 && n_tokens >= 0 && ldx >= K, "qt_xtx_accumulate_f32: bad arguments");
    QT_CHECK_ARG(K % 4 == 0 && ldx % 4 == 0 && ((uintptr_t)X & 15) == 0,
                 "qt_xtx_accumulate_f32: K, ldx must be multiples of 4 and X 16-byte aligned (K=%d)", K);
    if (n_tokens == 0) return QT_OK;
    const size_t need = qt_xtx_accumulate_f32_workspace_bytes(n_tokens, K);
    if (!workspace || workspace_bytes < need) {
        qt_set_error("qt_xtx_accumulate_f32: workspace %zu < required %zu", workspace_bytes, need);
        return QT_ERR_WORKSPACE;
    }
    const int64_t ldp = xf_pitch(K);
    const int64_t plane_stride = (int64_t)XF_CHUNK * ldp;
    char* ws = (char*)qt_align_up((size_t)workspace, 256);
    unsigned short* planes = (unsigned short*)ws;
    const size_t planes_bytes = (size_t)3 * XF_CHUNK * ldp * 2;
    char* tab = ws + planes_bytes;
    const int nt = (K + BT - 1) / BT;
    const size_t tab_bytes = qt_align_up((size_t)nt * (nt + 1) / 2 * sizeof(G3Item), 256);
    static std::mutex m;
    static std::map<std::pair<int, int>, G3Item*> tabs;
    auto table = [&](int nch) -> const G3Item* {
        std::lock_guard<std::mutex> lock(m);
        auto key = std::make_pair(K, nch);
        auto it = tabs.find(key);
        if (it != tabs.end()) return it->second;
        G3Item* pinned = nullptr;
        if (hipHostMalloc((void**)&pinned, tab_bytes, hipHostMallocDefault) != hipSuccess) return nullptr;
        int n = 0;
        for (int ti = 0; ti < nt; ++ti)
            for (int tj = 0; tj <= ti; ++tj) pinned[n++] = {(ti << 16) | tj, 0, nch, -1};
        tabs[key] = pinned;
        return pinned;
    };
    if (ldp != K) QT_HIP(hipMemsetAsync(planes, 0, planes_bytes, stream));
    int slot = 0;
    for (int64_t t0 = 0; t0 < n_tokens; t0 += XF_CHUNK) {
        const int rows = (int)std::min<int64_t>(XF_CHUNK, n_tokens - t0);
        const int rows_pad = (rows + 127) / 128 * 128;
        if (rows_pad != rows) {
            for (int q = 0; q < 3; ++q)
                QT_HIP(hipMemsetAsync(planes + q * plane_stride + (size_t)rows * ldp, 0, (size_t)(rows_pad - rows) * ldp * 2,
                                      stream));
        }
        int rc = qt_split3_launch(X + (size_t)t0 * ldx, ldx, rows, K, planes, ldp, plane_stride, 0, 0, 0, stream);
        if (rc) return rc;
        const int nch = rows_pad / CH_ROWS;
        const G3Item* host_tab = table(nch);
        if (!host_tab) {
            qt_set_error("qt_xtx_accumulate_f32: hipHostMalloc failed");
            return QT_ERR_HIP;
        }
        char* dev_tab = tab + (size_t)(slot & 1) * tab_bytes;
        ++slot;
        QT_HIP(hipMemcpyAsync(dev_tab, host_tab, (size_t)nt * (nt + 1) / 2 * sizeof(G3Item), hipMemcpyHostToDevice, stream));
        G3Args g;
        g.Apl = planes;
        g.Bpl = planes;
        g.plane_stride = plane_stride;
        g.ld = ldp;
        g.rowA0 = g.rowB0 = 0;
        g.colA0 = g.colB0 = 0;
        g.colmax = (int)ldp;
        g.M = K;
        g.N = K;
        g.C = G;
        g.ldc = K;
        g.mode = G3_ADD;
        g.slabs = nullptr;
        g.items = (const G3Item*)dev_tab;
        g.n_items = nt * (nt + 1) / 2;
        g.red = nullptr;
        g.n_red = 0;
        rc = qt_gemm3_launch(g, stream);
        if (rc) return rc;
    }
    return QT_OK;
}

extern "C" int qt_gemm3_plan_check(int Tm, int Tn, int c_end, int tri, int* n_items_out, int* n_slabs_out,
                                   int* longest_out) {
    if (Tm <= 0 || Tn <= 0 || c_end <= 0) return -1;
    std::vector<G3Item> items;
    std::vector<G3Red> red;
    g3_plan_row(Tm, Tn, c_end, tri, items, red);
    const int step = 256 / G3_CHUNK_ROWS;
    std::vector<int> cover((size_t)Tm * Tn * c_end, 0);
    std::vector<int> slab_seen;
    int longest = 0, n_slabs = 0;
    for (const G3Item& it : items) {
        const int ti = it.tile >> 16, tj = it.tile & 0xFFFF;
        if (ti >= Tm || tj >= Tn || it.c_lo >= it.c_hi || it.c_hi > c_end) return -2;
        const int lo = tri ? step * tj : 0;
        if (it.c_lo < lo) return -3;
        for (int c = it.c_lo; c < it.c_hi; ++c) cover[((size_t)ti * Tn + tj) * c_end + c]++;
        longest = std::max(longest, it.c_hi - it.c_lo);
        if (it.slab < 0) {
            if (it.c_lo != lo || it.c_hi != c_end) return -4;
        } else {
            if ((int)slab_seen.size() <= it.slab) slab_seen.resize(it.slab + 1, 0);
            if (slab_seen[it.slab]++) return -5;
            n_slabs = std::max(n_slabs, it.slab + 1);
        }
    }
    for (int ti = 0; ti < Tm; ++ti)
        for (int tj = 0; tj < Tn; ++tj)
            for (int c = 0; c < c_end; ++c) {
                const int want = (c >= (tri ? step * tj : 0)) ? 1 : 0;
                if (cover[((size_t)ti * Tn + tj) * c_end + c] != want) return -6;
            }
    std::vector<int> in_red(n_slabs, 0);
    for (const G3Red& r : red) {
        if (r.count < 2 || r.first < 0 || r.first + r.count > n_slabs) return -7;
        for (int q = 0; q < r.count; ++q)
            if (in_red[r.first + q]++) return -8;
        int prev_hi = -1;
        for (int q = 0; q < r.count; ++q) {
            bool found = false;
            for (const G3Item& it : items)
                if (it.slab == r.first + q) {
                    if (it.tile != r.tile || (prev_hi >= 0 && it.c_lo != prev_hi)) return -9;
                    prev_hi = it.c_hi;
                    found = true;
                }
            if (!found) return -10;
        }
    }
    for (int q = 0; q < n_slabs; ++q)
        if (!in_red[q]) return -11;
    long tiles = 0;
    for (int tj = 0; tj < Tn; ++tj) tiles += (c_end > (tri ? step * tj : 0)) ? Tm : 0;
    if (tiles <= NUM_CU && (long)items.size() > NUM_CU) return -12;
    if (n_items_out) *n_items_out = (int)items.size();
    if (n_slabs_out) *n_slabs_out = n_slabs;
    if (longest_out) *longest_out = longest;
    return 0;
}
```

quantool_amd/hip/_lib.py:

```python
from __future__ import annotations

import ctypes
from ctypes import c_char_p, c_double, c_float, c_int, c_int32, c_int64, c_size_t, c_void_p
from pathlib import Path

_PKG = Path(__file__).resolve().parent.parent
LIB_PATH = _PKG / "lib" / "libquantool_hip.so"

QT_OK = 0
QT_ERR_INVALID = -1
QT_ERR_NOT_PD = -2
QT_ERR_WORKSPACE = -3
QT_ERR_HIP = -4
QT_ERR_UNSUPPORTED = -5

QT_F32, QT_BF16, QT_F16 = 0, 1, 2
QT_W_INT8, QT_W_INT4_PACKED = 0, 1

SIGNATURES = {
    "qt_version": (c_int, []),
    "qt_last_error": (c_char_p, []),
    "qt_xtx_workspace_bytes": (c_size_t, [c_int64, c_int]),
    "qt_xtx_accumulate": (c_int, [c_void_p, c_int, c_int64, c_int, c_int64, c_void_p, c_void_p, c_size_t, c_void_p]),
    "qt_xtx_accumulate_f32_workspace_bytes": (c_size_t, [c_int64, c_int]),
    "qt_xtx_accumulate_f32": (c_int, [c_void_p, c_int64, c_int, c_int64, c_void_p, c_void_p, c_size_t, c_void_p]),
    "qt_act_stats_workspace_bytes": (c_size_t, [c_int64, c_int]),
    "qt_act_stats_accumulate": (c_int, [c_void_p, c_int, c_int64, c_int, c_int64, c_void_p, c_void_p, c_void_p,
                                        c_void_p, c_size_t, c_void_p]),
    "qt_hessian_prepare_workspace_bytes": (c_size_t, [c_int]),
    "qt_hessian_prepare": (c_int, [c_void_p, c_int, c_int64, c_float, c_void_p, c_void_p, c_void_p, c_void_p,
                                   c_void_p, c_size_t, c_void_p]),
    "qt_hessian_prepare_damp": (c_int, [c_void_p, c_int, c_int64, c_float, c_void_p, c_void_p, c_void_p, c_void_p,
                                        c_void_p, c_void_p, c_size_t, c_void_p]),
    "qt_hessian_diag": (c_int, [c_void_p, c_int, c_int64, c_void_p, c_void_p]),
    "qt_argsort_desc": (c_int, [c_void_p, c_int, c_void_p, c_void_p, c_void_p]),
    "qt_cholesky_inverse_upper_workspace_bytes": (c_size_t, [c_int]),
    "qt_cholesky_inverse_upper": (c_int, [c_void_p, c_int, c_void_p, c_void_p, c_void_p, c_size_t, c_void_p]),
    "qt_cholesky_inverse_upper_batched_workspace_bytes": (c_size_t, [c_int, c_int]),
    "qt_cholesky_inverse_upper_batched": (c_int, [c_void_p, c_int64, c_int, c_void_p, c_int64, c_void_p, c_int, c_void_p,
                                                  c_size_t, c_void_p]),
    "qt_cholesky_inverse_upper_bounded": (c_int, [c_void_p, c_int, c_void_p, c_void_p, c_void_p, c_void_p, c_size_t,
                                                  c_void_p]),
    "qt_cholesky_inverse_upper_batched_bounded": (c_int, [c_void_p, c_int64, c_int, c_void_p, c_int64, c_void_p, c_int,
                                                          c_void_p, c_void_p, c_size_t, c_void_p]),
    "qt_group_minmax_qparams": (c_int, [c_void_p, c_int, c_int, c_int, c_int64, c_int, c_int, c_int, c_void_p,
                                        c_void_p, c_void_p, c_void_p, c_void_p]),
    "qt_weight_gather_f32": (c_int, [c_void_p, c_int, c_int, c_int, c_int64, c_void_p, c_void_p, c_void_p,
                                     c_void_p]),
    "qt_weight_gather_qparams": (c_int, [c_void_p, c_int, c_int, c_int, c_int64, c_void_p, c_void_p, c_int, c_int, c_int,
                                         c_void_p, c_void_p, c_void_p, c_void_p, c_void_p, c_int64, c_void_p]),
    "qt_gptq_sweep_workspace_bytes": (c_size_t, [c_int, c_int, c_int]),
    "qt_gptq_sweep": (c_int, [c_void_p, c_int, c_int, c_void_p, c_void_p, c_void_p, c_int, c_void_p, c_int, c_int,
                              c_void_p, c_void_p, c_void_p, c_size_t, c_void_p]),
    "qt_gptq_sweep_grouped": (c_int, [c_void_p, c_int, c_int, c_void_p, c_int64, c_int, c_void_p, c_void_p, c_void_p, c_int,
                                      c_void_p, c_int, c_int, c_void_p, c_void_p, c_void_p, c_size_t, c_void_p]),
    "qt_pack_int4": (c_int, [c_void_p, c_int, c_int, c_void_p, c_void_p, c_void_p]),
    "qt_awq_weight_mean_workspace_bytes": (c_size_t, [c_int, c_int]),
    "qt_awq_weight_mean_accumulate": (c_int, [c_void_p, c_int, c_int, c_int, c_int64, c_int, c_void_p, c_void_p,
                                              c_size_t, c_void_p]),
    "qt_awq_scales": (c_int, [c_void_p, c_int64, c_void_p, c_int64, c_int, c_int, c_int, c_void_p, c_void_p]),
    "qt_symmetrize_lower": (c_int, [c_void_p, c_int, c_void_p]),
    "qt_awq_loss_workspace_bytes": (c_size_t, [c_int, c_int]),
    "qt_awq_loss": (c_int, [c_void_p, c_int, c_int, c_int, c_int64, c_void_p, c_int, c_int, c_int, c_void_p, c_int64,
                            c_int, c_float, c_int, c_void_p, c_void_p, c_size_t, c_void_p]),
    "qt_awq_losses_workspace_bytes": (c_size_t, [c_int, c_int, c_int]),
    "qt_awq_losses": (c_int, [c_void_p, c_int, c_int, c_int, c_int64, c_void_p, c_int, c_int, c_int, c_int, c_void_p,
                              c_int64, c_float, c_int, c_void_p, c_void_p, c_size_t, c_void_p]),
    "qt_argmin_f32": (c_int, [c_void_p, c_int, c_void_p, c_void_p]),
    "qt_awq_pseudo_quantize": (c_int, [c_void_p, c_int, c_int, c_int, c_int64, c_void_p, c_int, c_int, c_int, c_void_p,
                                       c_int64, c_void_p]),
    "qt_scale_columns": (c_int, [c_void_p, c_int, c_int, c_int, c_int64, c_void_p, c_int, c_void_p, c_int64,
                                 c_void_p]),
    "qt_rtn_quantize": (c_int, [c_void_p, c_int, c_int, c_int, c_int64, c_void_p, c_void_p, c_int, c_int, c_int,
                                c_void_p, c_void_p]),
    "qt_col_absmax_workspace_bytes": (c_size_t, [c_int, c_int]),
    "qt_col_absmax_accumulate": (c_int, [c_void_p, c_int, c_int, c_int, c_int64, c_void_p, c_void_p, c_size_t,
                                         c_void_p]),
    "qt_smoothquant_scales": (c_int, [c_void_p, c_void_p, c_void_p, c_int, c_float, c_void_p, c_void_p]),
    "qt_xtx_dot_workspace_bytes": (c_size_t, [c_int64, c_int]),
    "qt_xtx_dot": (c_int, [c_void_p, c_int, c_int64, c_int, c_int64, c_void_p, c_double, c_void_p, c_int, c_void_p,
                           c_size_t, c_void_p]),
    "qt_gemm3_plan_check": (c_int, [c_int, c_int, c_int, c_int, c_void_p, c_void_p, c_void_p]),
    "qt_xtx_tile_table_check": (c_int, [c_int, c_void_p, c_void_p, c_void_p]),
    "qt_gemm3_tn_f32_workspace_bytes": (c_size_t, [c_int, c_int, c_int]),
    "qt_gemm3_tn_f32": (c_int, [c_void_p, c_int64, c_void_p, c_int64, c_void_p, c_int64, c_int, c_int, c_int, c_int,
                                c_void_p, c_size_t, c_void_p]),
    "qt_gemm3_tn_f32_ex": (c_int, [c_void_p, c_int64, c_void_p, c_int64, c_void_p, c_int64, c_int, c_int, c_int, c_int,
                                   c_int, c_int, c_int, c_int64, c_int64, c_int64, c_void_p, c_size_t, c_void_p]),
    "qt_gemm3_tn_f16x2": (c_int, [c_void_p, c_int64, c_void_p, c_int64, c_void_p, c_int64, c_int, c_int, c_int, c_int,
                                  c_int, c_int, c_int, c_int64, c_int64, c_int64, c_void_p, c_void_p, c_void_p, c_size_t,
                                  c_void_p]),
    "qt_sgemm_tn_f32_workspace_bytes": (c_size_t, [c_int, c_int]),
    "qt_sgemm_tn_f32": (c_int, [c_void_p, c_int64, c_void_p, c_int64, c_void_p, c_int64, c_void_p, c_int64, c_int,
                                c_int, c_int, c_int, c_int, c_int, c_void_p, c_size_t, c_void_p]),
    "qt_profile_enable": (c_int, [c_int]),
    "qt_profile_read": (c_int, [c_int, c_void_p, c_void_p]),
    "qt_dequantize": (c_int, [c_void_p, c_int, c_int, c_void_p, c_void_p, c_void_p, c_int, c_void_p, c_void_p,
                              c_int, c_int64, c_void_p]),
    "qt_quantize_tokens_i8": (c_int, [c_void_p, c_int, c_int64, c_int, c_int64, c_void_p, c_int, c_void_p, c_void_p,
                                      c_void_p, c_void_p]),
    "qt_act_mul_quantize_i8": (c_int, [c_void_p, c_int64, c_void_p, c_int64, c_int, c_int64, c_int, c_int, c_void_p,
                                       c_int, c_void_p, c_void_p, c_void_p, c_void_p, c_int64, c_void_p]),
    "qt_rmsnorm_quantize_i8": (c_int, [c_void_p, c_int64, c_void_p, c_int, c_int64, c_int, c_float, c_void_p, c_int,
                                       c_void_p, c_void_p, c_void_p, c_void_p, c_int64, c_void_p, c_void_p]),
    "qt_gemm_i8": (c_int, [c_void_p, c_int64, c_int, c_void_p, c_int, c_int, c_void_p, c_void_p, c_void_p, c_int,
                           c_void_p, c_void_p, c_void_p, c_int, c_int64, c_void_p]),
    "qt_gemm_i8_skinny": (c_int, [c_void_p, c_int, c_int, c_void_p, c_int, c_int, c_void_p, c_void_p, c_void_p, c_int,
                                  c_void_p, c_void_p, c_void_p, c_int, c_int64, c_void_p]),
    "qt_gemm_i8_ring": (c_int, [c_void_p, c_int64, c_int, c_void_p, c_int, c_int, c_void_p, c_void_p, c_void_p, c_int,
                                c_void_p, c_void_p, c_void_p, c_int, c_int64, c_void_p]),
    "qt_gemm_i8_ring_w4": (c_int, [c_void_p, c_int64, c_int, c_void_p, c_int, c_int, c_void_p, c_void_p, c_void_p,
                                   c_int, c_void_p, c_void_p, c_void_p, c_int, c_int64, c_void_p]),
    "qt_gemm_i8_mid": (c_int, [c_void_p, c_int64, c_int, c_void_p, c_int, c_int, c_void_p, c_void_p, c_void_p, c_int,
                               c_void_p, c_void_p, c_void_p, c_int, c_int64, c_void_p]),
    "qt_gemm_i8_skinny_grouped": (c_int, [c_void_p, c_int, c_void_p, c_int64, c_void_p, c_int, c_void_p, c_int, c_int,
                                          c_void_p, c_void_p, c_void_p, c_int, c_void_p, c_void_p, c_int, c_int64,
                                          c_void_p]),
    "qt_moe_route": (c_int, [c_void_p, c_int, c_int64, c_int, c_int, c_void_p, c_void_p, c_void_p, c_void_p,
                             c_void_p]),
    "qt_gemm_i8_grouped": (c_int, [c_void_p, c_int, c_void_p, c_int64, c_void_p, c_int, c_void_p, c_int, c_int,
                                   c_void_p, c_void_p, c_void_p, c_int, c_void_p, c_void_p, c_int, c_int64, c_void_p]),
    "qt_gemm_i8_ring_grouped": (c_int, [c_void_p, c_int, c_void_p, c_int64, c_void_p, c_int, c_void_p, c_int, c_int,
                                        c_void_p, c_void_p, c_void_p, c_int, c_void_p, c_void_p, c_int, c_int64,
                                        c_int64, c_void_p]),
    "qt_moe_gemm_i8_ring_w4": (c_int, [c_void_p, c_int, c_void_p, c_int64, c_void_p, c_int, c_void_p, c_int, c_int,
                                       c_void_p, c_void_p, c_void_p, c_int, c_void_p, c_void_p, c_int, c_int64,
                                       c_int64, c_void_p]),
    "qt_moe_gemm_i8_wide": (c_int, [c_void_p, c_int, c_void_p, c_int64, c_void_p, c_int, c_void_p, c_int, c_int,
                                    c_void_p, c_void_p, c_void_p, c_int, c_void_p, c_void_p, c_int, c_int64,
                                    c_int64, c_void_p]),
    "qt_moe_combine": (c_int, [c_void_p, c_int, c_int, c_int64, c_void_p, c_void_p, c_int64, c_int, c_void_p,
                               c_void_p]),
    "qt_dequantize_weight": (c_int, [c_void_p, c_int, c_int, c_int, c_void_p, c_int, c_void_p, c_void_p, c_void_p,
                                     c_int, c_int64, c_void_p]),
    "qt_gemm_wq_skinny": (c_int, [c_void_p, c_int, c_int, c_int, c_int64, c_void_p, c_int, c_int, c_void_p, c_int,
                                  c_void_p, c_void_p, c_void_p, c_void_p, c_int64, c_void_p]),
    "qt_gemm_wq_stream": (c_int, [c_void_p, c_int, c_int, c_int, c_int64, c_void_p, c_int, c_int, c_void_p, c_int,
                                  c_void_p, c_void_p, c_void_p, c_void_p, c_int64, c_void_p]),
    "qt_gemm_wq_grouped": (c_int, [c_void_p, c_int, c_int, c_int64, c_void_p, c_int64, c_void_p, c_int, c_void_p,
                                   c_int, c_int, c_void_p, c_int, c_void_p, c_void_p, c_void_p, c_int64, c_void_p]),
    "qt_moe_gemm_wq_wide": (c_int, [c_void_p, c_int, c_int, c_int64, c_void_p, c_int64, c_void_p, c_int, c_void_p,
                                    c_int, c_int, c_void_p, c_int, c_void_p, c_void_p, c_void_p, c_int64, c_int64,
                                    c_void_p]),
}

_lib = None


class HipBackendError(RuntimeError):

    def __init__(self, fn: str, status: int, message: str):
        super().__init__(f"{fn} failed with status {status}: {message}")
        self.status = status


def load() -> ctypes.CDLL:
    global _lib
    if _lib is not None:
        return _lib
    if not LIB_PATH.exists():
        raise ImportError(
            f"quantool_amd HIP library not found at {LIB_PATH}. Build it with "
            "`python -c 'import __graft_entry__ as g; g.build()'` (needs hipcc). "
            "There is no CPU fallback for the quantization path."
        )
    import torch

    lib = ctypes.CDLL(str(LIB_PATH))
    for name, (res, args) in SIGNATURES.items():
        fn = getattr(lib, name)
        fn.restype = res
        fn.argtypes = args
    _lib = lib
    return lib


def check(fn_name: str, status: int) -> None:
    if status != QT_OK:
        msg = load().qt_last_error()
        raise HipBackendError(fn_name, status, msg.decode() if msg else "")
```

Baseline: 3.152 billion.

## Interleave Cholesky factor and inverse row steps, merging their GEMM3 launches

Restructures the blocked Cholesky-plus-triangular-inverse so that, for each outer block row, the trailing-update product and the inverse product are planned into a single gemm3 launch with two output segments, selected per tile by a segment bit. The factorization and inversion phases are interleaved per block row, and trinv runs per block range through a new blk0 offset. The goal is to halve the number of small gemm3 and reduce launches and to fill more CUs per launch. In exchange it adds a more complex planner, a slab budget tied to the separate plan, and extra branching in the kernel epilogue and reduce kernel.

```diff
diff --git a/include/quantool_amd.h b/include/quantool_amd.h
--- a/include/quantool_amd.h
+++ b/include/quantool_amd.h
@@ -142,6 +142,7 @@
                       qt_stream_t stream);
 
 int qt_gemm3_plan_check(int Tm, int Tn, int c_end, int tri, int* n_items_out, int* n_slabs_out, int* longest_out);
+int qt_chol_g3_plan_check(int K, int merged, int min_chunks, long long* counts_out);
 enum qt_act { QT_ACT_SILU = 0 };
 #define QT_I8_MID_MAX_M 128
 #define QT_I8_MID_K_UNIT 128
diff --git a/quantool_amd/csrc/cholesky.hip b/quantool_amd/csrc/cholesky.hip
--- a/quantool_amd/csrc/cholesky.hip
+++ b/quantool_amd/csrc/cholesky.hip
@@ -26,9 +26,11 @@
 struct CholG3Plan {
     bool any = false;
     std::vector<G3Step> fac, inv;
+    std::vector<G3Step> row;
     char* blob = nullptr;
     size_t blob_bytes = 0;
     int max_slabs = 0;
+    bool any_row = false;
 };
 
 static int chol_g3_min_chunks() {
@@ -45,23 +47,30 @@
     return K < 8192 ? 96 : 256;
 }
 
-static const CholG3Plan* chol_g3_plan(int K, int NBO, int NBI) {
-    static std::mutex m;
-    static std::map<std::tuple<int, int, int, int>, CholG3Plan*> plans;
-    const int min_chunks = chol_g3_min_chunks();
-    const int target_items = chol_g3_target_items(K);
-    std::lock_guard<std::mutex> lock(m);
-    const auto key = std::make_tuple(K, NBO, NBI, min_chunks * 1024 + target_items);
-    auto it = plans.find(key);
-    if (it != plans.end()) return it->second;
-    CholG3Plan* pl = new CholG3Plan();
-    std::vector<char> bytes;
-    auto add = [&](int Tm, int Tn, int c_end, int tri) {
+enum { CHOL_TWO_PHASE = 0, CHOL_WALK = 1, CHOL_WALK_MERGED = 2 };
+static int chol_merge_mode() {
+    const char* e = getenv("QT_CHOL_MERGE");
+    if (!e) return CHOL_WALK_MERGED;
+    if (strcmp(e, "order") == 0) return CHOL_WALK;
+    return atoi(e) != 0 ? CHOL_WALK_MERGED : CHOL_TWO_PHASE;
+}
+
+static void chol_g3_build(int K, int NBO, int NBI, int min_chunks, int target_items, bool merged, CholG3Plan& pl,
+                          std::vector<char>& bytes) {
+    pl = CholG3Plan();
+    bytes.clear();
+    int slab_budget = 0;
+    if (merged) {
+        CholG3Plan sep;
+        std::vector<char> sep_bytes;
+        chol_g3_build(K, NBO, NBI, min_chunks, target_items, false, sep, sep_bytes);
+        slab_budget = sep.max_slabs;
+    }
+    auto enough = [&](int Tm, int Tn, int c_end, int tri) {
+        return min_chunks > 0 && K % 8 == 0 && g3_row_chunks(Tm, Tn, c_end, tri) * G3_CHUNK_ROWS >= (long)min_chunks * 128;
+    };
+    auto store = [&](const std::vector<G3Item>& items, const std::vector<G3Red>& red) {
         G3Step st;
-        if (min_chunks <= 0 || K % 8 != 0 || g3_row_chunks(Tm, Tn, c_end, tri) * G3_CHUNK_ROWS < (long)min_chunks * 128) return st;
-        std::vector<G3Item> items;
-        std::vector<G3Red> red;
-        g3_plan_row(Tm, Tn, c_end, tri, items, red, target_items);
         st.n_items = (int)items.size();
         st.n_red = (int)red.size();
         st.item_off = qt_align_up(bytes.size(), 256);
@@ -70,20 +79,59 @@
         st.red_off = qt_align_up(bytes.size(), 256);
         bytes.resize(st.red_off + red.size() * sizeof(G3Red));
         if (!red.empty()) memcpy(bytes.data() + st.red_off, red.data(), red.size() * sizeof(G3Red));
-        for (const G3Red& r : red) pl->max_slabs = pl->max_slabs > r.first + r.count ? pl->max_slabs : r.first + r.count;
-        pl->any = true;
+        for (const G3Red& r : red) pl.max_slabs = pl.max_slabs > r.first + r.count ? pl.max_slabs : r.first + r.count;
+        pl.any = true;
         return st;
     };
-    for (int J0 = 0; J0 < K; J0 += NBO) {
+    auto add = [&](int Tm, int Tn, int c_end, int tri) {
+        if (!enough(Tm, Tn, c_end, tri)) return G3Step();
+        std::vector<G3Item> items;
+        std::vector<G3Red> red;
+        g3_plan_row(Tm, Tn, c_end, tri, items, red, target_items);
+        return store(items, red);
+    };
+    const bool walk = merged && NBO == NBI;
+    const int cap = target_items > 0 && target_items < 256 ? target_items : 256;
+    pl.row.assign(walk ? (K + NBO - 1) / NBO : 0, G3Step());
+    std::vector<char> is_merged(pl.row.size(), 0);
+    for (int J0 = 0, Jb = 0; J0 < K; J0 += NBO, ++Jb) {
         const int J1 = (K - J0 < NBO) ? K : J0 + NBO;
-        pl->fac.push_back(J0 == 0 ? G3Step() : add((J1 - J0 + 255) / 256, (K - J0 + 255) / 256, J0 / G3_CHUNK_ROWS, 0));
-    }
-    for (int I0 = 0; I0 < K; I0 += NBI) {
+        const int Tm = (J1 - J0 + 255) / 256, Tn0 = (K - J0 + 255) / 256, Tn1 = (J0 + 255) / 256, c_end = J0 / G3_CHUNK_ROWS;
+        if (walk && J0 > 0 && 2 * Tm * (Tn0 + Tn1) <= cap && enough(Tm, Tn0, c_end, 0) && enough(Tm, Tn1, c_end, 1)) {
+            std::vector<G3Item> items;
+            std::vector<G3Red> red;
+            g3_plan_row2(Tm, Tn0, Tn1, c_end, items, red, target_items, slab_budget);
+            pl.row[Jb] = store(items, red);
+            is_merged[Jb] = 1;
+            pl.any_row = true;
+        }
+    }
+    for (int J0 = 0, Jb = 0; J0 < K; J0 += NBO, ++Jb) {
+        const int J1 = (K - J0 < NBO) ? K : J0 + NBO;
+        const bool skip = J0 == 0 || (walk && is_merged[Jb]);
+        pl.fac.push_back(skip ? G3Step() : add((J1 - J0 + 255) / 256, (K - J0 + 255) / 256, J0 / G3_CHUNK_ROWS, 0));
+    }
+    for (int I0 = 0, Ib = 0; I0 < K; I0 += NBI, ++Ib) {
         const int I1 = (K - I0 < NBI) ? K : I0 + NBI;
-        pl->inv.push_back(I0 == 0 ? G3Step() : add((I1 - I0 + 255) / 256, (I0 + 255) / 256, I0 / G3_CHUNK_ROWS, 1));
-    }
+        const bool skip = I0 == 0 || (walk && is_merged[Ib]);
+        pl.inv.push_back(skip ? G3Step() : add((I1 - I0 + 255) / 256, (I0 + 255) / 256, I0 / G3_CHUNK_ROWS, 1));
+    }
+    pl.blob_bytes = pl.any ? qt_align_up(bytes.size(), 256) : 0;
+}
+
+static const CholG3Plan* chol_g3_plan(int K, int NBO, int NBI, bool merged = false) {
+    static std::mutex m;
+    static std::map<std::tuple<int, int, int, int>, CholG3Plan*> plans;
+    const int min_chunks = chol_g3_min_chunks();
+    const int target_items = chol_g3_target_items(K);
+    std::lock_guard<std::mutex> lock(m);
+    const auto key = std::make_tuple(K, NBO, NBI, (merged ? 1 << 30 : 0) + min_chunks * 1024 + target_items);
+    auto it = plans.find(key);
+    if (it != plans.end()) return it->second;
+    CholG3Plan* pl = new CholG3Plan();
+    std::vector<char> bytes;
+    chol_g3_build(K, NBO, NBI, min_chunks, target_items, merged, *pl, bytes);
     if (pl->any) {
-        pl->blob_bytes = qt_align_up(bytes.size(), 256);
         if (hipHostMalloc((void**)&pl->blob, pl->blob_bytes, hipHostMallocDefault) != hipSuccess) {
             pl->any = false;
             pl->blob = nullptr;
@@ -96,6 +144,7 @@
         pl->max_slabs = 0;
         for (G3Step& st : pl->fac) st = G3Step();
         for (G3Step& st : pl->inv) st = G3Step();
+        for (G3Step& st : pl->row) st = G3Step();
     }
     plans[key] = pl;
     return pl;
@@ -351,7 +400,8 @@
 
 __global__ __launch_bounds__(128) void trinv_batched_kernel(const float* __restrict__ Rd_all, int K,
                                                             float* __restrict__ Dinv_all,
-                                                            float* __restrict__ Y, int64_t ldy, int64_t bsW, int64_t bsY) {
+                                                            float* __restrict__ Y, int64_t ldy, int64_t bsW, int64_t bsY,
+                                                            int blk0) {
     if (blockIdx.y) {
         Rd_all += (size_t)blockIdx.y * bsW;
         Dinv_all += (size_t)blockIdx.y * bsW;
@@ -360,7 +410,7 @@
     extern __shared__ __attribute__((aligned(16))) float sm[];
     float* Rt = sm;
     float* Xs = sm + NB * LDT;
-    const int b = blockIdx.x;
+    const int b = blk0 + blockIdx.x;
     const int n = (K - b * NB < NB) ? K - b * NB : NB;
     const float* Rd = Rd_all + (size_t)b * RD_STRIDE;
     const int j = threadIdx.x;
@@ -421,14 +471,15 @@
 
 __global__ __launch_bounds__(256) void trinv_mfma_kernel(const float* __restrict__ Rd_all, int K,
                                                          float* __restrict__ Dinv_all,
-                                                         float* __restrict__ Y, int64_t ldy, int64_t bsW, int64_t bsY) {
+                                                         float* __restrict__ Y, int64_t ldy, int64_t bsW, int64_t bsY,
+                                                         int blk0) {
     if (blockIdx.y) {
         Rd_all += (size_t)blockIdx.y * bsW;
         Dinv_all += (size_t)blockIdx.y * bsW;
         Y += (size_t)blockIdx.y * bsY;
     }
     extern __shared__ __attribute__((aligned(16))) float Rs[];
-    const int blk = blockIdx.x;
+    const int blk = blk0 + blockIdx.x;
     const int n = (K - blk * NB < NB) ? K - blk * NB : NB;
     const float* Rd = Rd_all + (size_t)blk * RD_STRIDE;
     const int tid = threadIdx.x, lane = tid & 63, wave = tid >> 6;
@@ -606,6 +657,15 @@
     char* ws = (char*)qt_align_up((size_t)workspace, 256);
     int NBO, NBI;
     const CholG3Plan* g3 = chol_blocks(K, NBO, NBI);
+    int merge_mode = (g3->any && NBO == NBI) ? chol_merge_mode() : CHOL_TWO_PHASE;
+    const CholG3Plan* tab = g3;
+    if (merge_mode == CHOL_WALK_MERGED) {
+        tab = chol_g3_plan(K, NBO, NBI, true);
+        if (!tab->any || !tab->any_row || tab->max_slabs > g3->max_slabs || tab->blob_bytes > g3->blob_bytes) {
+            tab = g3;
+            merge_mode = CHOL_TWO_PHASE;
+        }
+    }
     const size_t prob_bytes = chol_problem_ws_bytes(K, g3);
     const int64_t sW = (int64_t)(prob_bytes / 4);
     const int64_t sA = nprob > 1 ? strideA : 0, sU = nprob > 1 ? strideU : 0;
@@ -628,14 +688,14 @@
         q += qt_align_up((size_t)3 * K * K * 2, 256);
         g3_slabs = (float*)q;
         g3_tab = (char*)qt_align_up((size_t)(ws + (size_t)nprob * prob_bytes), 256);
-        QT_HIP(hipMemcpyAsync(g3_tab, g3->blob, g3->blob_bytes, hipMemcpyHostToDevice, stream));
+        QT_HIP(hipMemcpyAsync(g3_tab, tab->blob, tab->blob_bytes, hipMemcpyHostToDevice, stream));
     }
     f16x2 = f16x2 && g3->any;
     int32_t* eR = f16x2 ? (int32_t*)(Rpl + 2 * plane_stride) : nullptr;
     int32_t* eY = f16x2 ? eR + nprob : nullptr;
     static_assert(2 * SG_MAX_BATCH * sizeof(int32_t) <= (size_t)NB * NB * 2, "the exponents fit the smallest third plane");
     auto g3_row = [&](const G3Step& st, const unsigned short* Bplanes, int col_a0, int col_b0, int M, int N, float* C,
-                      int64_t bsC, int mode) -> int {
+                      int64_t bsC, int mode, bool second = false) -> int {
         G3Args a;
         a.Apl = Rpl;
         a.Bpl = Bplanes;
@@ -663,6 +723,16 @@
             a.planes = G3_F16X2;
             a.eA = eR;
             a.eB = Bplanes == Rpl ? eR : eY;
+        }
+        if (second) {
+            a.Bpl1 = Ypl;
+            a.colB01 = 0;
+            a.eB1 = eY;
+            a.C1 = TI;
+            a.ldc1 = K;
+            a.bsC1 = sW;
+            a.mode1 = G3_SET;
+            a.N1 = col_a0;
         }
         return qt_gemm3_launch(a, stream);
     };
@@ -700,26 +770,21 @@
         QT_LAUNCH_CHECK();
     }
 
-    for (int J0 = 0, Jb = 0; J0 < K; J0 += NBO, ++Jb) {
-        const int J1 = (K - J0 < NBO) ? K : J0 + NBO;
-        if (g3->any && J0 > 0) {
-            const G3Step& st = g3->fac[Jb];
-            float* C = A + (size_t)J0 * K + J0;
-            if (st.n_items > 0) {
-                int rc = g3_row(st, Rpl, J0, J0, J1 - J0, K - J0, C, sA, G3_SUB);
-                if (rc) return rc;
-            } else {
-                SgemmArgs g;
-                g.A = A + J0; g.lda = K;
-                g.B = A + J0; g.ldb = K;
-                g.Cin = C; g.ldcin = K;
-                g.Cout = C; g.ldcout = K;
-                g.M = J1 - J0; g.N = K - J0; g.kdim = J0; g.k_mode = SG_K_FULL; g.mode = SG_MODE_SUB;
-                g.split_ws = split_ws; g.split_ws_bytes = split_ws_bytes;
-                int rc = sgemm(g, sA, sA, sA);
-                if (rc) return rc;
-            }
-        }
+    auto fac_product = [&](int J0, int J1, int Jb) -> int {
+        if (!(g3->any && J0 > 0)) return QT_OK;
+        const G3Step& st = tab->fac[Jb];
+        float* C = A + (size_t)J0 * K + J0;
+        if (st.n_items > 0) return g3_row(st, Rpl, J0, J0, J1 - J0, K - J0, C, sA, G3_SUB);
+        SgemmArgs g;
+        g.A = A + J0; g.lda = K;
+        g.B = A + J0; g.ldb = K;
+        g.Cin = C; g.ldcin = K;
+        g.Cout = C; g.ldcout = K;
+        g.M = J1 - J0; g.N = K - J0; g.kdim = J0; g.k_mode = SG_K_FULL; g.mode = SG_MODE_SUB;
+        g.split_ws = split_ws; g.split_ws_bytes = split_ws_bytes;
+        return sgemm(g, sA, sA, sA);
+    };
+    auto fac_panels = [&](int J0, int J1) -> int {
         for (int j0 = J0; j0 < J1; j0 += NB) {
             const int j = j0 / NB, nbj = (K - j0 < NB) ? K - j0 : NB;
             float* Ajj = A + (size_t)j0 * K + j0;
@@ -764,19 +829,32 @@
             int rc = sgemm(g, sA, sA, sA);
             if (rc) return rc;
         }
-    }
-    {
+        return QT_OK;
+    };
+    auto trinv = [&](int blk0, int n) -> int {
         const char* e = getenv("QT_CHOL_TRINV");
         if (e && strcmp(e, "div") == 0)
-            hipLaunchKernelGGL(trinv_batched_kernel, dim3(nblk, nprob), dim3(NB), inv_lds, stream, (const float*)Rd, K, Dinv, Y,
-                               (int64_t)K, sW, sY);
+            hipLaunchKernelGGL(trinv_batched_kernel, dim3(n, nprob), dim3(NB), inv_lds, stream, (const float*)Rd, K, Dinv, Y,
+                               (int64_t)K, sW, sY, blk0);
         else
-            hipLaunchKernelGGL(trinv_mfma_kernel, dim3(nblk, nprob), dim3(256), RD_STRIDE * sizeof(float), stream,
-                               (const float*)Rd, K, Dinv, Y, (int64_t)K, sW, sY);
-    }
-    QT_LAUNCH_CHECK();
-    for (int I0 = 0, Ib = 0; I0 < K; I0 += NBI, ++Ib) {
-        const int I1 = (K - I0 < NBI) ? K : I0 + NBI;
+            hipLaunchKernelGGL(trinv_mfma_kernel, dim3(n, nprob), dim3(256), RD_STRIDE * sizeof(float), stream,
+                               (const float*)Rd, K, Dinv, Y, (int64_t)K, sW, sY, blk0);
+        QT_LAUNCH_CHECK();
+        return QT_OK;
+    };
+    auto inv_product = [&](int I0, int I1, int Ib) -> int {
+        if (I0 == 0) return QT_OK;
+        if (g3->any && tab->inv[Ib].n_items > 0) return g3_row(tab->inv[Ib], Ypl, I0, 0, I1 - I0, I0, TI, sW, G3_SET);
+        SgemmArgs g;
+        g.A = A + I0; g.lda = K;
+        g.B = Y; g.ldb = K;
+        g.Cin = nullptr; g.ldcin = 0;
+        g.Cout = TI; g.ldcout = K;
+        g.M = I1 - I0; g.N = I0; g.kdim = I0; g.k_mode = SG_K_FROM_N0; g.mode = SG_MODE_SET;
+        g.split_ws = split_ws; g.split_ws_bytes = split_ws_bytes;
+        return sgemm(g, sA, sY, sW);
+    };
+    auto inv_row = [&](int I0, int I1) -> int {
         const int Wi = I1 - I0;
         for (int i0 = I0 + NB; i0 < I1; i0 += NB) {
             const int i = i0 / NB, nbi = (K - i0 < NB) ? K - i0 : NB;
@@ -805,25 +883,7 @@
             return qt_split3_launch(Y + (size_t)I0 * K, K, Wi, I1, Ypl + (size_t)I0 * K, K, plane_stride, 1, I0, 0, stream,
                                     nprob, sY, sW * 2);
         };
-        if (I0 == 0) {
-            int rc0 = split_row();
-            if (rc0) return rc0;
-            continue;
-        }
-        int rc;
-        if (g3->any && g3->inv[Ib].n_items > 0) {
-            rc = g3_row(g3->inv[Ib], Ypl, I0, 0, Wi, I0, TI, sW, G3_SET);
-        } else {
-            SgemmArgs g;
-            g.A = A + I0; g.lda = K;
-            g.B = Y; g.ldb = K;
-            g.Cin = nullptr; g.ldcin = 0;
-            g.Cout = TI; g.ldcout = K;
-            g.M = Wi; g.N = I0; g.kdim = I0; g.k_mode = SG_K_FROM_N0; g.mode = SG_MODE_SET;
-            g.split_ws = split_ws; g.split_ws_bytes = split_ws_bytes;
-            rc = sgemm(g, sA, sY, sW);
-        }
-        if (rc) return rc;
+        if (I0 == 0) return split_row();
         hipLaunchKernelGGL(transpose_lower_block_kernel, dim3((Wi + 31) / 32, (Wi + 31) / 32, nprob), dim3(256), 0, stream,
                            (const float*)(Y + (size_t)I0 * K + I0), (int64_t)K, Wi, XT, NBO_MAX, sY, sW);
         QT_LAUNCH_CHECK();
@@ -833,10 +893,40 @@
         t.Cin = nullptr; t.ldcin = 0;
         t.Cout = Y + (size_t)I0 * K; t.ldcout = K;
         t.M = Wi; t.N = I0; t.kdim = Wi; t.k_mode = SG_K_FULL; t.mode = SG_MODE_NEG;
-        rc = sgemm(t, sW, sW, sY);
+        int rc = sgemm(t, sW, sW, sY);
         if (rc) return rc;
-        rc = split_row();
+        return split_row();
+    };
+    if (merge_mode == CHOL_TWO_PHASE) {
+        for (int J0 = 0, Jb = 0; J0 < K; J0 += NBO, ++Jb) {
+            const int J1 = (K - J0 < NBO) ? K : J0 + NBO;
+            int rc = fac_product(J0, J1, Jb);
+            if (!rc) rc = fac_panels(J0, J1);
+            if (rc) return rc;
+        }
+        int rc = trinv(0, nblk);
         if (rc) return rc;
+        for (int I0 = 0, Ib = 0; I0 < K; I0 += NBI, ++Ib) {
+            const int I1 = (K - I0 < NBI) ? K : I0 + NBI;
+            rc = inv_product(I0, I1, Ib);
+            if (!rc) rc = inv_row(I0, I1);
+            if (rc) return rc;
+        }
+    } else {
+        for (int J0 = 0, Jb = 0; J0 < K; J0 += NBO, ++Jb) {
+            const int J1 = (K - J0 < NBO) ? K : J0 + NBO;
+            int rc;
+            if (merge_mode == CHOL_WALK_MERGED && tab->row[Jb].n_items > 0) {
+                rc = g3_row(tab->row[Jb], Rpl, J0, J0, J1 - J0, K - J0, A + (size_t)J0 * K + J0, sA, G3_SUB, true);
+            } else {
+                rc = fac_product(J0, J1, Jb);
+                if (!rc) rc = inv_product(J0, J1, Jb);
+            }
+            if (!rc) rc = fac_panels(J0, J1);
+            if (!rc) rc = trinv(J0 / NB, (J1 - J0 + NB - 1) / NB);
+            if (!rc) rc = inv_row(J0, J1);
+            if (rc) return rc;
+        }
     }
     hipLaunchKernelGGL(flat_reverse_lower_to_upper_kernel, dim3((K + 255) / 256, K, nprob), dim3(256), 0, stream, U, K, sU);
     QT_LAUNCH_CHECK();
@@ -877,3 +967,90 @@
                  "qt_cholesky_inverse_upper_batched_bounded: strides must be multiples of 4 elements and >= K*K");
     return chol_run(A, strideA, K, U, strideU, info, n_problems, workspace, workspace_bytes, (hipStream_t)stream_, min_eig_lb);
 }
+
+extern "C" int qt_chol_g3_plan_check(int K, int merged, int min_chunks, long long* counts_out) {
+    if (K <= 0) return -1;
+    constexpr int NBX = 512, TRI_STEP = 256 / G3_CHUNK_ROWS;
+    if (min_chunks <= 0) min_chunks = 64;
+    const int cap = chol_g3_target_items(K);
+    CholG3Plan sep, pl;
+    std::vector<char> sep_bytes, bytes;
+    chol_g3_build(K, NBX, NBX, min_chunks, cap, false, sep, sep_bytes);
+    chol_g3_build(K, NBX, NBX, min_chunks, cap, merged != 0, pl, bytes);
+    if (pl.max_slabs > sep.max_slabs || pl.blob_bytes > sep.blob_bytes) return -2;
+    long long launches = 0, n_items = 0, n_slabs = 0;
+    auto check = [&](const G3Step& st, int Tm, int Tn0, int tri0, int Tn1, int c_end) -> int {
+        if (st.n_items <= 0) return 0;
+        const G3Item* items = (const G3Item*)(bytes.data() + st.item_off);
+        const G3Red* red = (const G3Red*)(bytes.data() + st.red_off);
+        if (st.n_items > cap && st.n_items > Tm * (Tn0 + Tn1)) return -3;
+        const int Tn[2] = {Tn0, Tn1};
+        auto lo_of = [&](int seg, int tj) { return (seg == 1 || tri0) ? TRI_STEP * tj : 0; };
+        std::vector<int> cover((size_t)2 * Tm * (Tn0 + Tn1 + 1) * c_end, 0);
+        auto cell = [&](int seg, int ti, int tj, int c) { return (((size_t)seg * Tm + ti) * (Tn0 + Tn1 + 1) + tj) * c_end + c; };
+        std::vector<int> owner(sep.max_slabs, -1);
+        int slabs_here = 0;
+        for (int q = 0; q < st.n_items; ++q) {
+            const G3Item& it = items[q];
+            const int seg = (it.tile & G3_SEG_BIT) ? 1 : 0, ti = it.tile >> 16, tj = it.tile & G3_TJ_MASK;
+            if (ti < 0 || ti >= Tm || tj >= Tn[seg]) return -4;
+            const int lo = lo_of(seg, tj);
+            if (it.c_lo < lo || it.c_hi > c_end || it.c_hi - it.c_lo < 2) return -5;
+            for (int c = it.c_lo; c < it.c_hi; ++c) cover[cell(seg, ti, tj, c)]++;
+            if (it.slab < 0) {
+                if (it.c_lo != lo || it.c_hi != c_end) return -6;
+            } else {
+                if (it.slab >= sep.max_slabs) return -7;
+                if (owner[it.slab] >= 0) return -8;
+                owner[it.slab] = q;
+                ++slabs_here;
+            }
+        }
+        for (int seg = 0; seg < 2; ++seg)
+            for (int ti = 0; ti < Tm; ++ti)
+                for (int tj = 0; tj < Tn[seg]; ++tj)
+                    for (int c = 0; c < c_end; ++c)
+                        if (cover[cell(seg, ti, tj, c)] != (c >= lo_of(seg, tj) ? 1 : 0)) return -9;
+        int in_red = 0;
+        for (int r = 0; r < st.n_red; ++r) {
+            const G3Red& e = red[r];
+            if (e.count < 2 || e.first < 0 || e.first + e.count > sep.max_slabs || (e.seg != 0 && e.seg != 1)) return -10;
+            const int want_tile = e.tile | (e.seg ? G3_SEG_BIT : 0);
+            int prev_hi = lo_of(e.seg, e.tile & G3_TJ_MASK);
+            for (int q = 0; q < e.count; ++q) {
+                const int o = owner[e.first + q];
+                if (o < 0 || items[o].tile != want_tile || items[o].c_lo != prev_hi) return -11;
+                prev_hi = items[o].c_hi;
+                owner[e.first + q] = -2;
+            }
+            if (prev_hi != c_end) return -12;
+            in_red += e.count;
+        }
+        if (in_red != slabs_here) return -13;
+        ++launches;
+        n_items += st.n_items;
+        n_slabs += slabs_here;
+        return 0;
+    };
+    for (int J0 = 0, Jb = 0; J0 < K; J0 += NBX, ++Jb) {
+        const int J1 = (K - J0 < NBX) ? K : J0 + NBX;
+        const int Tm = (J1 - J0 + 255) / 256, Tn0 = (K - J0 + 255) / 256, Tn1 = (J0 + 255) / 256, c_end = J0 / G3_CHUNK_ROWS;
+        int rc = 0;
+        if (Jb < (int)pl.row.size() && pl.row[Jb].n_items > 0) {
+            if (pl.fac[Jb].n_items > 0 || pl.inv[Jb].n_items > 0) return -14;
+            rc = check(pl.row[Jb], Tm, Tn0, 0, Tn1, c_end);
+        } else {
+            rc = check(pl.fac[Jb], Tm, Tn0, 0, 0, c_end);
+            if (!rc) rc = check(pl.inv[Jb], Tm, Tn1, 1, 0, c_end);
+        }
+        if (rc) return rc;
+    }
+    if (counts_out) {
+        counts_out[0] = launches;
+        counts_out[1] = n_items;
+        counts_out[2] = n_slabs;
+        counts_out[3] = sep.max_slabs;
+        counts_out[4] = (long long)pl.blob_bytes;
+    }
+    return 0;
+}
diff --git a/quantool_amd/csrc/gemm3_tn.h b/quantool_amd/csrc/gemm3_tn.h
--- a/quantool_amd/csrc/gemm3_tn.h
+++ b/quantool_amd/csrc/gemm3_tn.h
@@ -15,8 +15,10 @@
     int tile;
     int first;
     int count;
-    int pad;
+    int seg;
 };
+constexpr int G3_SEG_BIT = 1 << 15;
+constexpr int G3_TJ_MASK = G3_SEG_BIT - 1;
 
 enum { G3_SUB = 0, G3_SET = 1, G3_ADD = 2 };
 
@@ -47,6 +49,13 @@
     int planes = G3_BF16X3;
     const int32_t* eA = nullptr;
     const int32_t* eB = nullptr;
+    const unsigned short* Bpl1 = nullptr;
+    int colB01 = 0;
+    const int32_t* eB1 = nullptr;
+    float* C1 = nullptr;
+    int64_t ldc1 = 0, bsC1 = 0;
+    int mode1 = G3_SET;
+    int N1 = 0;
 };
 
 int qt_gemm3_launch(const G3Args& a, hipStream_t stream);
@@ -63,3 +72,5 @@
 
 long g3_row_chunks(int Tm, int Tn, int c_end, int tri);
 void g3_plan_row(int Tm, int Tn, int c_end, int tri, std::vector<G3Item>& items, std::vector<G3Red>& red, int target_items = 0);
+void g3_plan_row2(int Tm, int Tn0, int Tn1, int c_end, std::vector<G3Item>& items, std::vector<G3Red>& red,
+                  int target_items = 0, int max_slabs = 0);
diff --git a/quantool_amd/csrc/gemm3_tn.hip b/quantool_amd/csrc/gemm3_tn.hip
--- a/quantool_amd/csrc/gemm3_tn.hip
+++ b/quantool_amd/csrc/gemm3_tn.hip
@@ -44,6 +44,11 @@
     int64_t bsA_bytes, bsB_bytes, bsC, bsSlabs;
     const int32_t* eA;
     const int32_t* eB;
+    const char* Bpl1;
+    const int32_t* eB1;
+    float* C1;
+    int64_t ldc1, bsC1;
+    int colB01, N1, mode1;
 };
 
 template <int MODE, int LOOP>
@@ -56,25 +61,27 @@
     const int wave_m = wave >> 2, wave_n = wave & 3;
     const bool group_b = wave >= 4;
 
+    const G3Item* itp = p.items + blockIdx.x;
+    const int it_tile = __builtin_amdgcn_readfirstlane(itp->tile);
+    const bool seg1 = (it_tile & G3_SEG_BIT) != 0;
+    const char* Bpl = seg1 ? p.Bpl1 : p.Bpl;
+    const int colB0 = seg1 ? p.colB01 : p.colB0;
     if (blockIdx.y) {
         p.Apl += (size_t)blockIdx.y * p.bsA_bytes;
-        p.Bpl += (size_t)blockIdx.y * p.bsB_bytes;
-        p.C += (size_t)blockIdx.y * p.bsC;
+        Bpl += (size_t)blockIdx.y * p.bsB_bytes;
         p.slabs += (size_t)blockIdx.y * p.bsSlabs;
     }
-    const G3Item* itp = p.items + blockIdx.x;
-    const int it_tile = __builtin_amdgcn_readfirstlane(itp->tile);
     const int c_lo = __builtin_amdgcn_readfirstlane(itp->c_lo);
     const int c_hi = __builtin_amdgcn_readfirstlane(itp->c_hi);
     const int slab_idx = __builtin_amdgcn_readfirstlane(itp->slab);
-    const int ti = it_tile >> 16, tj = it_tile & 0xFFFF;
+    const int ti = it_tile >> 16, tj = it_tile & G3_TJ_MASK;
     const int nu = (c_hi - c_lo) * (LOOP != LOOP_CHUNK ? CH_ROWS / UT : CH_UNITS);
 
     const int rsub = lane >> 4;
     const int lch = (lane & 15) ^ (rsub << 2);
     const int trow = 4 * (wave & 3) + rsub;
     int colA = p.colA0 + ti * BT + (wave >> 2) * 128 + lch * 8;
-    int colB = p.colB0 + tj * BT + (wave >> 2) * 128 + lch * 8;
+    int colB = colB0 + tj * BT + (wave >> 2) * 128 + lch * 8;
     colA = colA > p.colmax - 8 ? p.colmax - 8 : colA;
     colB = colB > p.colmaxB - 8 ? p.colmaxB - 8 : colB;
     const unsigned voffA = (unsigned)((size_t)trow * (size_t)p.ld2 + (size_t)colA * 2);
@@ -104,7 +111,7 @@
 
     if constexpr (LOOP == LOOP_DUO) {
         const char* runA = p.Apl + (p.rowA0 + (int64_t)c_lo * CH_ROWS) * p.ld2;
-        const char* runB = p.Bpl + (p.rowB0 + (int64_t)c_lo * CH_ROWS) * p.ld2B;
+        const char* runB = Bpl + (p.rowB0 + (int64_t)c_lo * CH_ROWS) * p.ld2B;
         auto issue2 = [&](int slot) {
             const unsigned d = dst_wave + (unsigned)slot * DUO_BYTES;
 #pragma unroll
@@ -146,7 +153,7 @@
             for (int u = 0; u < nu; u += DRING) ring_body<DRING>(phase, u);
             ring_stagger_end(group_b);
         }
-        const int es = -(11 + p.eA[blockIdx.y] + p.eB[blockIdx.y]);
+        const int es = -(11 + p.eA[blockIdx.y] + (seg1 ? p.eB1 : p.eB)[blockIdx.y]);
         const float unscale = __builtin_bit_cast(float, (unsigned)(127 + (es < -126 ? -126 : es > 127 ? 127 : es)) << 23);
 #pragma unroll
         for (int mi = 0; mi < 4; ++mi)
@@ -156,7 +163,7 @@
                 for (int r = 0; r < 16; ++r) acc[mi][ni][r] *= unscale;
     } else if constexpr (TRI) {
         const char* runA = p.Apl + (p.rowA0 + (int64_t)c_lo * CH_ROWS) * p.ld2;
-        const char* runB = p.Bpl + (p.rowB0 + (int64_t)c_lo * CH_ROWS) * p.ld2B;
+        const char* runB = Bpl + (p.rowB0 + (int64_t)c_lo * CH_ROWS) * p.ld2B;
         auto issue3 = [&](int slot) {
             const unsigned d = dst_wave + (unsigned)slot * TRI_BYTES;
 #pragma unroll
@@ -216,7 +223,7 @@
             const int64_t plA = (PA_BITS >> (2 * pr)) & 3u, plB = (PB_BITS >> (2 * pr)) & 3u;
             const int64_t row = (int64_t)(c_lo + c) * CH_ROWS + j * UT;
             a = p.Apl + plA * p.plane_bytes + (p.rowA0 + row) * p.ld2;
-            b = p.Bpl + plB * p.plane_bytesB + (p.rowB0 + row) * p.ld2B;
+            b = Bpl + plB * p.plane_bytesB + (p.rowB0 + row) * p.ld2B;
         };
         auto issue = [&](int i, int slot) {
             const char *a, *b;
@@ -273,22 +280,32 @@
 
     const int jl = lane & 31, ih = 4 * (lane >> 5);
     if (slab_idx < 0) {
-#pragma unroll
-        for (int mi = 0; mi < 4; ++mi)
-#pragma unroll
-            for (int ni = 0; ni < 2; ++ni) {
-                const int gj = tj * BT + wave_n * 64 + ni * 32 + jl;
-#pragma unroll
-                for (int r = 0; r < 16; ++r) {
-                    const int gi = ti * BT + wave_m * 128 + mi * 32 + (r & 3) + 8 * (r >> 2) + ih;
-                    if (gi < p.M && gj < p.N) {
-                        float* dst = p.C + (size_t)gi * p.ldc + gj;
-                        if (MODE == G3_SUB) *dst = *dst - acc[mi][ni][r];
-                        else if (MODE == G3_ADD) *dst = *dst + acc[mi][ni][r];
-                        else *dst = acc[mi][ni][r];
+        float* C = (seg1 ? p.C1 : p.C) + (size_t)blockIdx.y * (size_t)(seg1 ? p.bsC1 : p.bsC);
+        const int64_t ldc = seg1 ? p.ldc1 : p.ldc;
+        const int N = seg1 ? p.N1 : p.N;
+        auto apply = [&](auto mode_c) {
+            constexpr int M_ = decltype(mode_c)::value;
+#pragma unroll
+            for (int mi = 0; mi < 4; ++mi)
+#pragma unroll
+                for (int ni = 0; ni < 2; ++ni) {
+                    const int gj = tj * BT + wave_n * 64 + ni * 32 + jl;
+#pragma unroll
+                    for (int r = 0; r < 16; ++r) {
+                        const int gi = ti * BT + wave_m * 128 + mi * 32 + (r & 3) + 8 * (r >> 2) + ih;
+                        if (gi < p.M && gj < N) {
+                            float* dst = C + (size_t)gi * ldc + gj;
+                            if (M_ == G3_SUB) *dst = *dst - acc[mi][ni][r];
+                            else if (M_ == G3_ADD) *dst = *dst + acc[mi][ni][r];
+                            else *dst = acc[mi][ni][r];
+                        }
                     }
                 }
-            }
+        };
+        const int mode = seg1 ? p.mode1 : MODE;
+        if (mode == G3_SUB) apply(std::integral_constant<int, G3_SUB>{});
+        else if (mode == G3_ADD) apply(std::integral_constant<int, G3_ADD>{});
+        else apply(std::integral_constant<int, G3_SET>{});
     } else {
         float* slab = p.slabs + (size_t)slab_idx * (size_t)(BT * BT);
 #pragma unroll
@@ -306,12 +323,20 @@
 
 __global__ __launch_bounds__(256) void gemm3_reduce_kernel(const float* __restrict__ slabs,
                                                            const G3Red* __restrict__ red, float* C, int64_t ldc,
-                                                           int M, int N, int mode, int64_t bsSlabs, int64_t bsC) {
+                                                           int M, int N, int mode, int64_t bsSlabs, int64_t bsC,
+                                                           float* C1, int64_t ldc1, int N1, int mode1, int64_t bsC1) {
+    const G3Red t = red[blockIdx.x];
+    if (t.seg) {
+        C = C1;
+        ldc = ldc1;
+        N = N1;
+        mode = mode1;
+        bsC = bsC1;
+    }
     if (blockIdx.z) {
         slabs += (size_t)blockIdx.z * bsSlabs;
         C += (size_t)blockIdx.z * bsC;
     }
-    const G3Red t = red[blockIdx.x];
     const int ti = t.tile >> 16, tj = t.tile & 0xFFFF;
     const int part = blockIdx.y;
     const size_t tile_elems = (size_t)BT * BT;
@@ -451,6 +476,18 @@
                  "qt_gemm3_launch: plane mode %d needs its scale exponents", a.planes);
     p.eA = a.eA;
     p.eB = a.eB;
+    const bool two = a.Bpl1 != nullptr;
+    QT_CHECK_ARG(!two || (((uintptr_t)a.Bpl1 & 15) == 0 && a.C1 && a.N1 > 0 && (a.planes != G3_F16X2 || a.eB1) &&
+                          a.mode1 >= G3_SUB && a.mode1 <= G3_ADD),
+                 "qt_gemm3_launch: second segment incomplete");
+    p.Bpl1 = two ? (const char*)a.Bpl1 : p.Bpl;
+    p.eB1 = two ? a.eB1 : a.eB;
+    p.C1 = two ? a.C1 : a.C;
+    p.ldc1 = two ? a.ldc1 : a.ldc;
+    p.bsC1 = two ? a.bsC1 : a.bsC;
+    p.colB01 = two ? a.colB01 : a.colB0;
+    p.N1 = two ? a.N1 : a.N;
+    p.mode1 = two ? a.mode1 : a.mode;
     const dim3 grid(a.n_items, nb);
     const char* loop_env = getenv("QT_G3_LOOP");
     const bool chunk_loop = loop_env && strcmp(loop_env, "chunk") == 0;
@@ -466,7 +503,7 @@
     QT_LAUNCH_CHECK();
     if (a.n_red > 0) {
         hipLaunchKernelGGL(gemm3_reduce_kernel, dim3(a.n_red, 16, nb), dim3(256), 0, stream, (const float*)a.slabs, a.red,
-                           a.C, a.ldc, a.M, a.N, a.mode, a.bsSlabs, a.bsC);
+                           a.C, a.ldc, a.M, a.N, a.mode, a.bsSlabs, a.bsC, p.C1, p.ldc1, p.N1, p.mode1, p.bsC1);
         QT_LAUNCH_CHECK();
     }
     return QT_OK;
@@ -507,39 +544,73 @@
     return total;
 }
 
-void g3_plan_row(int Tm, int Tn, int c_end, int tri, std::vector<G3Item>& items, std::vector<G3Red>& red, int target_items) {
-    constexpr int TRI_STEP = 256 / G3_CHUNK_ROWS;
+namespace {
+struct G3PlanTile {
+    int tile, lo, seg;
+};
+void g3_deal_xcds(std::vector<G3Item>& items);
+void g3_plan_tiles(const std::vector<G3PlanTile>& tiles, int c_end, std::vector<G3Item>& items, std::vector<G3Red>& red,
+                   int target_items, int max_slabs) {
     items.clear();
     red.clear();
-    const long total = g3_row_chunks(Tm, Tn, c_end, tri);
+    long total = 0;
+    for (const G3PlanTile& t : tiles) total += std::max(0, c_end - t.lo);
     const int cap = target_items > 0 && target_items < NUM_CU ? target_items : NUM_CU;
-    auto count_items = [&](int per) {
+    auto count_items = [&](int per, long& n_slabs) {
         long n_items = 0;
-        for (int tj = 0; tj < Tn; ++tj) {
-            const int n = c_end - (tri ? TRI_STEP * tj : 0);
-            if (n > 0) n_items += (long)Tm * ((n + per - 1) / per);
+        n_slabs = 0;
+        for (const G3PlanTile& t : tiles) {
+            const int n = c_end - t.lo;
+            if (n <= 0) continue;
+            const int pieces = (n + per - 1) / per;
+            n_items += pieces;
+            if (pieces > 1) n_slabs += pieces;
         }
         return n_items;
     };
     int per = std::max(2, (int)((total + cap - 1) / cap));
-    while (count_items(per) > cap && per < c_end) ++per;
+    long n_slabs = 0;
+    while ((count_items(per, n_slabs) > cap || (max_slabs > 0 && n_slabs > max_slabs)) && per < c_end) ++per;
     int next_slab = 0;
+    for (const G3PlanTile& t : tiles) {
+        const int lo = t.lo, n = c_end - lo;
+        if (n <= 0) continue;
+        const int pieces = (n + per - 1) / per;
+        if (pieces == 1) {
+            items.push_back({t.tile, lo, c_end, -1});
+            continue;
+        }
+        red.push_back({t.tile & ~G3_SEG_BIT, next_slab, pieces, t.seg});
+        for (int s = 0; s < pieces; ++s) {
+            const int a = lo + (int)((long)n * s / pieces), b = lo + (int)((long)n * (s + 1) / pieces);
+            items.push_back({t.tile, a, b, next_slab++});
+        }
+    }
+    g3_deal_xcds(items);
+}
+}
+
+void g3_plan_row(int Tm, int Tn, int c_end, int tri, std::vector<G3Item>& items, std::vector<G3Red>& red, int target_items) {
+    constexpr int TRI_STEP = 256 / G3_CHUNK_ROWS;
+    std::vector<G3PlanTile> tiles;
     for (int ti = 0; ti < Tm; ++ti)
-        for (int tj = 0; tj < Tn; ++tj) {
-            const int lo = tri ? TRI_STEP * tj : 0, n = c_end - lo;
-            if (n <= 0) continue;
-            const int pieces = (n + per - 1) / per;
-            const int tile = (ti << 16) | tj;
-            if (pieces == 1) {
-                items.push_back({tile, lo, c_end, -1});
-                continue;
-            }
-            red.push_back({tile, next_slab, pieces, 0});
-            for (int s = 0; s < pieces; ++s) {
-                const int a = lo + (int)((long)n * s / pieces), b = lo + (int)((long)n * (s + 1) / pieces);
-                items.push_back({tile, a, b, next_slab++});
-            }
-        }
+        for (int tj = 0; tj < Tn; ++tj) tiles.push_back({(ti << 16) | tj, tri ? TRI_STEP * tj : 0, 0});
+    g3_plan_tiles(tiles, c_end, items, red, target_items, 0);
+}
+
+void g3_plan_row2(int Tm, int Tn0, int Tn1, int c_end, std::vector<G3Item>& items, std::vector<G3Red>& red, int target_items,
+                  int max_slabs) {
+    constexpr int TRI_STEP = 256 / G3_CHUNK_ROWS;
+    std::vector<G3PlanTile> tiles;
+    for (int ti = 0; ti < Tm; ++ti)
+        for (int tj = 0; tj < Tn0; ++tj) tiles.push_back({(ti << 16) | tj, 0, 0});
+    for (int ti = 0; ti < Tm; ++ti)
+        for (int tj = 0; tj < Tn1; ++tj) tiles.push_back({(ti << 16) | G3_SEG_BIT | tj, TRI_STEP * tj, 1});
+    g3_plan_tiles(tiles, c_end, items, red, target_items, max_slabs);
+}
+
+namespace {
+void g3_deal_xcds(std::vector<G3Item>& items) {
     std::stable_sort(items.begin(), items.end(),
                      [](const G3Item& x, const G3Item& y) { return (x.c_hi - x.c_lo) > (y.c_hi - y.c_lo); });
     static const bool deal = [] { const char* e = getenv("QT_G3_DEAL"); return !(e && atoi(e) == 0); }();
@@ -563,6 +634,7 @@
                 if (q < cls[x].size()) dealt.push_back(cls[x][q]);
         items.swap(dealt);
     }
+}
 }
 
 int g3_scale_exponent(float bound) {
diff --git a/quantool_amd/hip/_lib.py b/quantool_amd/hip/_lib.py
--- a/quantool_amd/hip/_lib.py
+++ b/quantool_amd/hip/_lib.py
@@ -82,6 +82,7 @@
                            c_size_t, c_void_p]),
     "qt_gemm3_plan_check": (c_int, [c_int, c_int, c_int, c_int, c_void_p, c_void_p, c_void_p]),
     "qt_xtx_tile_table_check": (c_int, [c_int, c_void_p, c_void_p, c_void_p]),
+    "qt_chol_g3_plan_check": (c_int, [c_int, c_int, c_int, c_void_p]),
     "qt_gemm3_tn_f32_workspace_bytes": (c_size_t, [c_int, c_int, c_int]),
     "qt_gemm3_tn_f32": (c_int, [c_void_p, c_int64, c_void_p, c_int64, c_void_p, c_int64, c_int, c_int, c_int, c_int,
                                 c_void_p, c_size_t, c_void_p]),
```

New measurement: 3.221 billion (median of 6 runs). 1.02x the previous value.
